# thallolang/thallo

Hardware: AMD Instinct MI355X
Metric: pcg_iters_per_sec (higher is better)
Workload: dtype f32

## Files before the change

include/thallo_hip.h:

```cpp
#ifndef THALLO_HIP_H
#define THALLO_HIP_H

#ifdef __cplusplus
extern "C" {
#endif

typedef void* thallo_stream_t;

#define THALLO_HIP_MAX_PARTIALS 1024

typedef struct thallo_sum_t {
    const float* partials;
    int          count;
} thallo_sum_t;

typedef struct thallo_segs_t {
    long off[8];
    long len[8];
    int  n;
} thallo_segs_t;

#define THALLO_DIST_MAX_WORLD 8
#define THALLO_DIST_CTL_WORDS 16
typedef struct thallo_dist_t {
    unsigned long long* mail;
    unsigned long long* peer_mail[THALLO_DIST_MAX_WORLD];
    float*    peer_r[2];
    long      peer_off_o[2];
    long      peer_off_a[2];
    unsigned* ctl;
    int       world, rank;
} thallo_dist_t;

typedef struct thallo_fin_t {
    thallo_sum_t alphaN;
    unsigned*    tickets;
    float*       alphaD_word;
    float*       betaN_word;
} thallo_fin_t;

typedef struct thallo_prev_t {
    const float*  alphaD_partials;
    const double* s12_partials;
    int           count;
    float*        alphaD_word;
    float*        betaN_word;
} thallo_prev_t;

long thallo_hip_vector_elems(long n_unknowns);
int  thallo_hip_device_cu_count(void);


int thallo_hip_pcg_step2(float* r, const float* Ap, const float* pre, float* z, long n,
                         thallo_sum_t alphaN, thallo_sum_t alphaD, float* betaN_out, thallo_stream_t stream);

int thallo_hip_pcg_step2_ranges(float* r, const float* Ap, const float* pre, float* z,
                                long off0, long len0, long off1, long len1,
                                thallo_sum_t alphaN, thallo_sum_t alphaD, float* betaN_out, thallo_stream_t stream);

int thallo_hip_pcg_step2_full(float* delta, const float* p, float* r, const float* Ap, const float* pre,
                              float* z, const float* b, long n, thallo_sum_t alphaN, thallo_sum_t alphaD,
                              float* betaN_out, float* q_out, int lm, thallo_stream_t stream);

int thallo_hip_pcg_step3(float* p, const float* z, long n, thallo_sum_t betaN, thallo_sum_t alphaN,
                         int lm, thallo_stream_t stream);

int thallo_hip_pcg_pupdate(const float* z, const float* p_in, float* p_out, float* delta, long n, int first,
                           thallo_sum_t alphaN_prev, thallo_sum_t alphaD_prev, thallo_sum_t betaN_prev, thallo_stream_t stream);
int thallo_hip_pcg_pupdate_ranges(const float* z, const float* p_in, float* p_out, float* delta,
                                  long off0, long len0, long off1, long len1, int first,
                                  thallo_sum_t alphaN_prev, thallo_sum_t alphaD_prev, thallo_sum_t betaN_prev, thallo_stream_t stream);

int thallo_hip_lm_finalize_diagonal(const float* diag, float* SSq, float* CtC, float* pre, const float* r, float* b, float* z, long n,
                                    float radius, float min_lm_diagonal, float max_lm_diagonal, int save_ssq, int use_preconditioner,
                                    float* alphaN_out, thallo_stream_t stream);
int thallo_hip_lm_step1_finish(float* Ap, const float* CtC, const float* p, long n, float* alphaD_out, thallo_stream_t stream);
int thallo_hip_lm_step2_first_half(float* delta, const float* p, long n, thallo_sum_t alphaN, thallo_sum_t alphaD, thallo_stream_t stream);
int thallo_hip_lm_step2_second_half(float* r, const float* b, const float* Adelta, const float* pre, float* z, const float* delta, long n,
                                    float* betaN_out, float* q_out, thallo_stream_t stream);
int thallo_hip_pcg_init_finish(const float* r, const float* diag, float* pre, float* z, long n, int use_preconditioner,
                               float* alphaN_out, thallo_stream_t stream);
void thallo_hip_lm_set_gate(const unsigned* gate);
int thallo_hip_lm_state_reset(float* state, thallo_stream_t stream);
int thallo_hip_lm_zeta(thallo_sum_t q, int k, float q_tolerance, float* state, thallo_stream_t stream);
int thallo_hip_pcg_step2_full_zeta(float* delta, const float* p, float* r, const float* Ap, const float* pre,
                                   float* z, const float* b, long n, thallo_sum_t alphaN, thallo_sum_t alphaD,
                                   float* betaN_out, float* q_out, unsigned* tickets, int k, float q_tolerance, float* lm_state, thallo_stream_t stream);
int thallo_hip_dot(const float* a, const float* b, long n, float* out, thallo_stream_t stream);

int thallo_hip_linear_update(float* X, const float* delta, const float* p, long len,
                             thallo_sum_t alphaN, thallo_sum_t alphaD, thallo_stream_t stream);

int thallo_hip_slab_pack_iter(const float* vec, thallo_segs_t segs, const float* alphaD_partials, const double* s3_partials, int count, float* out, thallo_stream_t stream);
int thallo_hip_slab_unpack_iter(float* vec, thallo_segs_t top, const float* src_top, thallo_segs_t bot, const float* src_bot,
                                const float* gathered, long stride, int world, thallo_sum_t alphaN, float* alphaD_word, float* betaN_word, thallo_stream_t stream);
int thallo_hip_block_sums(const float* p, const float* Ap, const float* r, const float* pre, long n, float* alphaD_out, double* s3_out, thallo_stream_t stream);
int thallo_hip_shard_scalars(const float* gathered, long stride, int world, const float* alphaD_partials, const double* s3_partials, int count, thallo_sum_t alphaN,
                             float* alphaD_word, float* betaN_word, thallo_stream_t stream);
int thallo_hip_range_unpack(float* vec, thallo_segs_t first_rank_pieces, const float* gathered, long stride, long skip, int world, thallo_stream_t stream);
int thallo_hip_linear_update2(float* X, const float* delta, const float* p_older, thallo_sum_t alphaN_older, thallo_sum_t alphaD_older,
                              const float* p, thallo_sum_t alphaN, thallo_sum_t alphaD, long len, thallo_stream_t stream);
#define THALLO_HIP_MAX_UPDATE_TERMS 32
typedef struct { const float* p[THALLO_HIP_MAX_UPDATE_TERMS]; thallo_sum_t alphaN[THALLO_HIP_MAX_UPDATE_TERMS], alphaD[THALLO_HIP_MAX_UPDATE_TERMS]; int count; } thallo_update_terms_t;
int thallo_hip_linear_update_n(float* X, float* delta, thallo_update_terms_t terms, long len, int max_workgroups , thallo_stream_t stream);
int thallo_hip_linear_update_n_from_zero(float* X, float* delta, thallo_update_terms_t terms, long len, int max_workgroups, thallo_stream_t stream);
int thallo_hip_wave64_selftest(unsigned long long* out_ballot, unsigned* out_peers, float* sums4);
int thallo_hip_finish_sum(thallo_sum_t s, float* out, thallo_stream_t stream);
int thallo_hip_finish_sum_gated(thallo_sum_t s, float* out, const unsigned* gate, thallo_stream_t stream);

int thallo_hip_slab_pack(const float* vec, thallo_segs_t segs, thallo_sum_t sum, float* out, thallo_stream_t stream);
int thallo_hip_slab_unpack(float* vec, thallo_segs_t top, const float* src_top, thallo_segs_t bot, const float* src_bot,
                           const float* gathered, long stride, int world, float* sum_out, thallo_stream_t stream);

int thallo_hip_alpha_beta(thallo_sum_t alphaN, thallo_sum_t alphaD, thallo_sum_t betaN, float* out2,
                          thallo_stream_t stream);

int thallo_hip_lapimg_cost(int W, int H, const float* X, const float* A, float w_fit, int xguard,
                           float* cost_out, thallo_stream_t stream);
int thallo_hip_lapimg_pcg_init(int W, int H, const float* X, const float* A, float w_fit, int xguard,
                               float* r, float* z, float* p_prev, float* delta,
                               float* diag_out, float* alphaN_out, thallo_stream_t stream);
int thallo_hip_lapimg_apply_jtj(int W, int H, float w_fit, int xguard, const float* p, float* Ap, float* alphaD_out, thallo_stream_t stream);
int thallo_hip_lapimg_pcg_step1(int W, int H, float w_fit, int xguard,
                                const float* z, const float* p_in, float* p_out, float* delta, float* Ap,
                                int first, thallo_sum_t alphaN_prev, thallo_sum_t alphaD_prev, thallo_sum_t betaN_prev,
                                float* alphaD_out, thallo_stream_t stream);

int thallo_hip_iw_cost(int W, int H, int row0, int row1, const float* offset, const float* angle, const float* urshape,
                       const float* constraints, const float* mask, float w_fit, float w_reg,
                       float* cost_out, thallo_stream_t stream);
int thallo_hip_iw_pcg_init(int W, int H, int row0, int row1, const float* offset, const float* angle, const float* urshape,
                           const float* constraints, const float* mask, float w_fit, float w_reg,
                           float* r, float* pre, float* z, float* p_prev, float* delta,
                           float* cs, unsigned char* flags, float* diag_out, int* irregular_out, float* alphaN_out, thallo_stream_t stream);
int thallo_hip_iw_pcg_step1(int W, int H, int row0, int row1, const float* cs, const float* urshape, const unsigned char* flags,
                            float w_fit, float w_reg,
                            const float* z, const float* p_in, float* p_out, float* delta, float* Ap,
                            int mode, thallo_sum_t alphaN_prev, thallo_sum_t alphaD_prev, thallo_sum_t betaN_prev,
                            thallo_sum_t alphaN_prev2, thallo_sum_t alphaD_prev2,
                            const int* irregular, const float* r, float* alphaD_out, thallo_stream_t stream);
#define THALLO_IW_STEP1_MODE(k, batched) ((k) == 0 ? 1 : !(batched) ? 0 : ((k) & 1) ? 2 : 4)
#define THALLO_HIP_FIN_TICKET_WORDS 528
typedef struct thallo_iw_iter_t {
    int W, H, row0, row1;
    const float* cs;
    const float* urshape;
    const unsigned char* flags;
    const float* pre;
    const int* irregular;
    float w_fit, w_reg;
    const float* r_in;  float* r_out;
    const float* Ap_in; float* Ap_out;
    const float* p_in;  float* p_out;
    float* delta;
    int mode;
    thallo_sum_t alphaN_prev, alphaD_prev, betaN_prev, alphaN_prev2, alphaD_prev2;
    float* alphaD_out; double* s12_out;
    unsigned* fin_tickets; float* alphaD_word; float* betaN_word; int slot0;
    const thallo_dist_t* dist;
    const thallo_prev_t* prev;
    int prev_slot0; unsigned long long* gs;
} thallo_iw_iter_t;
unsigned thallo_hip_iw_iter_size(void);
enum { THALLO_IW_ITER_TILE = 0, THALLO_IW_ITER_MARCH = 1, THALLO_IW_ITER_MARCH_RC = 2 };
int thallo_hip_iw_pcg_iter(int kernel, const thallo_iw_iter_t* a, thallo_stream_t stream);
int thallo_hip_iw_march_rc_deferred_fits(int W, int rows);
int thallo_hip_iw_dist_finish_deferred(thallo_prev_t prev, int prev_slot0, thallo_sum_t alphaN_prev, thallo_dist_t d, unsigned long long* gs, thallo_stream_t stream);
void thallo_hip_march_rc_debug_set(int what, int value);
int thallo_hip_iw_urshape_irregular(int W, int H, const float* urshape, int* count_out, thallo_stream_t stream);
void thallo_hip_march_debug_set(int what, int value);
int  thallo_hip_iw_resident_rows(int W, int rows);
long thallo_hip_iw_resident_bytes(int W, int rows);
int  thallo_hip_iw_pcg_resident(int W, int H, int row0, int row1, const float* cs, const unsigned char* flags, float w_fit, float w_reg,
                                const float* r_in, const float* p_in, float* r_out, float* Ap_out, float* p_out, float* delta,
                                thallo_sum_t alphaN0, float* words, const int* irregular, float* X_offset, float* X_angle, void* xbuf, int L, thallo_stream_t stream);
int  thallo_hip_iw_resident_status(void* xbuf, int clear, int spin_ms, unsigned* pm, thallo_stream_t stream);
int  thallo_hip_iw_resident_rows_slab(int W, int rows, int below);
long thallo_hip_iw_resident_ghost_bytes(int W);
int  thallo_hip_iw_pcg_resident_dist(int W, int H, int row0, int row1, const float* cs, const unsigned char* flags, float w_fit, float w_reg,
                                     const float* r_in, const float* p_in, float* r_out, float* Ap_out, float* p_out, float* delta,
                                     thallo_sum_t alphaN0, float* words, const int* irregular, void* xbuf, thallo_dist_t d, long ghost_off, int slot0, int L, thallo_stream_t stream);
void thallo_hip_resident_debug_set(int what, int value);
int thallo_hip_iw_march_rows(int W, int rows);
int thallo_hip_iw_march_place(int W, int row0, int row1, int R, int grid, int* place);
int thallo_hip_iw_pcg_iter_finish(const float* alphaD_partials, const double* s12_partials, int count, thallo_sum_t alphaN,
                                  float* alphaD_word, float* betaN_word, thallo_stream_t stream);

int thallo_hip_iw_pcg_step2(int W, int H, int row0, int row1, const unsigned char* flags, float w_fit, float w_reg,
// ... 369 lines not shown
```

thallo_amd/csrc/energy_image_warping.hip:

```cpp
#include "iw_device.hpp"

using namespace thallo;

namespace {

constexpr int TW = 64, TH = 16, BLOCK = 256;
constexpr int LW = TW + 2, LH = TH + 2, LN = LW * LH;
constexpr int PER = TH / (BLOCK / TW);
constexpr int HALO = 2 * LW + 2 * TH;

inline Geo make_geo(int W, int H, int row0, int row1)
{
    Geo g; g.W = W; g.H = H; g.row0 = row0; g.row1 = row1;
    g.tx = (W + TW - 1) / TW; g.ty = (row1 - row0 + TH - 1) / TH; g.ntiles = g.tx * g.ty;
    return g;
}
inline bool rows_ok(int H, int row0, int row1) { return row0 >= 0 && row1 <= H && row0 < row1; }
inline int grid_for(const Geo& g, int per_cu)
{
    int cap = thallo_hip_device_cu_count() * per_cu;
    if (cap > THALLO_MAX_PARTIALS) cap = THALLO_MAX_PARTIALS;
    cap -= cap % 8;
    return g.ntiles < cap ? g.ntiles : cap;
}
// ... 228 lines not shown
        const long i = in_off ? off0 + j : off1 + (j - len0);
        float4 rv = ldf4(r + i, true);
        const float4 av = Ap[i];
        rv.x -= alpha * av.x; rv.y -= alpha * av.y; rv.z -= alpha * av.z; rv.w -= alpha * av.w;
        float4 m;
        if (grid) {
            if (in_off) {
                const unsigned f2 = reinterpret_cast<const unsigned short*>(flags)[i];
                float m0, m1, dummy;
                pre_from_flags((unsigned char)(f2 & 255), wf2, wr2, m0, dummy); pre_from_flags((unsigned char)(f2 >> 8), wf2, wr2, m1, dummy);
                m = make_float4(m0, m0, m1, m1);
            } else {
                const unsigned f4 = reinterpret_cast<const unsigned*>(flags)[i - N / 2];
                float d, a0, a1, a2, a3;
                pre_from_flags((unsigned char)(f4 & 255), wf2, wr2, d, a0); pre_from_flags((unsigned char)((f4 >> 8) & 255), wf2, wr2, d, a1);
                pre_from_flags((unsigned char)((f4 >> 16) & 255), wf2, wr2, d, a2); pre_from_flags((unsigned char)(f4 >> 24), wf2, wr2, d, a3);
                m = make_float4(a0, a1, a2, a3);
            }
        } else m = pre[i];
        const float4 zv = make_float4(m.x * rv.x, m.y * rv.y, m.z * rv.z, m.w * rv.w);
        stf4(r + i, rv, true);
        if (!grid) z[i] = zv;
        if (DIST) {
            const long jj = in_off ? j : j - len0, rowlen = in_off ? row_o4 : row_a4, total = in_off ? len0 : len1;
            if (jj < rowlen && dd.peer_r[0]) {
                float* dst = dd.peer_r[0] + (in_off ? dd.peer_off_o[0] : dd.peer_off_a[0]) + 4 * jj;
                st_sys(dst, rv.x); st_sys(dst + 1, rv.y); st_sys(dst + 2, rv.z); st_sys(dst + 3, rv.w);
            }
            if (jj >= total - rowlen && dd.peer_r[1]) {
                float* dst = dd.peer_r[1] + (in_off ? dd.peer_off_o[1] : dd.peer_off_a[1]) + 4 * (jj - (total - rowlen));
                st_sys(dst, rv.x); st_sys(dst + 1, rv.y); st_sys(dst + 2, rv.z); st_sys(dst + 3, rv.w);
            }
        }
        acc += zv.x * rv.x + zv.y * rv.y + zv.z * rv.z + zv.w * rv.w;
    }
    block_store_partial(acc, bN_out, red);
}

__global__ __launch_bounds__(BLOCK) void k_step2_iw_rows(float* __restrict__ r, const float* __restrict__ Ap, const float* __restrict__ pre, float* __restrict__ z,
                                                         long off0, long len0, long off1, long len1, thallo_sum_t aN, thallo_sum_t aD, float* __restrict__ bN_out)
{
    __shared__ float red[16];
    const float alpha = safe_div<false>(sum_partials(aN.partials, aN.count), sum_partials(aD.partials, aD.count));
    float acc = 0.0f;
    const long n = len0 + len1;
    for (long j = (long)blockIdx.x * BLOCK + threadIdx.x; j < n; j += (long)gridDim.x * BLOCK) {
        const long i = j < len0 ? off0 + j : off1 + (j - len0);
        const float rv = r[i] - alpha * Ap[i];
        const float zv = pre ? pre[i] * rv : rv;
        r[i] = rv; z[i] = zv;
        acc += zv * rv;
    }
    block_store_partial(acc, bN_out, red);
}

__global__ __launch_bounds__(BLOCK) void k_init(Geo g, const float2* __restrict__ off, const float* __restrict__ ang,
                                                const float2* __restrict__ ur, const float2* __restrict__ cons,
                                                const float* __restrict__ mask, float wf, float wr,
                                                float* __restrict__ r, float* __restrict__ pre, float* __restrict__ z,
                                                float* __restrict__ p_prev, float* __restrict__ delta,
                                                float2* __restrict__ cs, unsigned char* __restrict__ flags,
                                                float* __restrict__ diag_out, int* __restrict__ irregular, float* __restrict__ aN_out)
{
    __shared__ Tile T;
    __shared__ float red[16];
    const long N = (long)g.W * g.H;
    const float wr2 = wr * wr, wf2 = wf * wf;
    float acc = 0.0f;
    int bad = 0;
    for (TileSweep t(g.ntiles); t.valid(); t.next()) {
        const int x0 = (t.cur % g.tx) * TW, y0 = g.row0 + (t.cur / g.tx) * TH;
        for (int idx = threadIdx.x; idx < LN; idx += BLOCK) {
            const int ly = idx / LW, lx = idx - ly * LW;
            const int gx = x0 + lx - 1, gy = y0 + ly - 1;
            float ox = 0.f, oy = 0.f, cc = 1.f, ss = 0.f, uxx = 0.f, uyy = 0.f; unsigned char ff = 0;
            if (gx >= 0 && gx < g.W && gy >= 0 && gy < g.H) {
                const long pix = (long)gy * g.W + gx;
                const float2 o = off[pix]; const float2 u = ur[pix];
                ox = o.x; oy = o.y; uxx = u.x; uyy = u.y;
                sincosf(ang[pix], &ss, &cc);
                ff = mask[pix] == 0.0f ? 1 : 0;
                if ((gy < g.row0 || gy >= g.row1) && lx >= 1 && lx <= TW) {
                    cs[pix] = make_float2(cc, ss); flags[pix] = ff;
                    reinterpret_cast<float2*>(p_prev)[pix] = make_float2(0.f, 0.f); p_prev[2 * N + pix] = 0.f;
                }
            }
            T.px[idx] = ox; T.py[idx] = oy; T.c[idx] = cc; T.s[idx] = ss; T.ux[idx] = uxx; T.uy[idx] = uyy; T.f[idx] = ff;
        }
        __syncthreads();
        const int lx = (threadIdx.x % TW) + 1;
        const int gx = x0 + lx - 1;
        for (int k = 0; k < PER; ++k) {
            const int ly = (threadIdx.x / TW) * PER + k + 1;
            const int gy = y0 + ly - 1;
            const int i = ly * LW + lx;
            if (gx < g.W && gy < g.row1) {
                const long pix = (long)gy * g.W + gx;
                const unsigned char act = T.f[i] & 1;
                const bool bad_x = gx + 1 < g.W && (T.ux[i + 1] - T.ux[i] != 1.0f || T.uy[i + 1] - T.uy[i] != 0.0f);
                const bool bad_y = gy + 1 < g.H && (T.ux[i + LW] - T.ux[i] != 0.0f || T.uy[i + LW] - T.uy[i] != 1.0f);
                if (bad_x || bad_y) ++bad;
                float rx = 0.f, ry = 0.f, ra = 0.f, mx = 0.f, my = 0.f, ma = 0.f, dgo_raw = 0.f, dga_raw = 0.f;
                unsigned char fl = act;
                if (act) {
                    const float oxi = T.px[i], oyi = T.py[i], ci = T.c[i], si = T.s[i], uxi = T.ux[i], uyi = T.uy[i];
                    float jx = 0.f, jy = 0.f, ja = 0.f, dgo = 0.f, dga = 0.f;
                    int cnt = 0; bool unit = true;
                    const int nb[4] = { i + 1, i - 1, i + LW, i - LW };
#pragma unroll
                    for (int d = 0; d < 4; ++d) {
                        const int j = nb[d];
                        if (T.f[j] & 1) {
                            const float dux = uxi - T.ux[j], duy = uyi - T.uy[j];
                            unit = unit && dux == (d == 0 ? -1.0f : d == 1 ? 1.0f : 0.0f) && duy == (d == 2 ? -1.0f : d == 3 ? 1.0f : 0.0f);
                            ++cnt;
                            const float dox = oxi - T.px[j], doy = oyi - T.py[j];
                            const float eix = dox - (ci * dux - si * duy), eiy = doy - (si * dux + ci * duy);
                            const float cj = T.c[j], sj = T.s[j];
                            const float ejx = -dox + (cj * dux - sj * duy), ejy = -doy + (sj * dux + cj * duy);
                            const float gix = -si * dux - ci * duy, giy = ci * dux - si * duy;
                            jx += eix - ejx; jy += eiy - ejy;
                            ja -= gix * eix + giy * eiy;
                            dgo += 2.0f; dga += gix * gix + giy * giy;
                        }
                    }
                    jx *= wr2; jy *= wr2; ja *= wr2; dgo *= wr2; dga *= wr2;
                    if (unit) dga = (float)cnt * wr2;
                    fl |= (unsigned char)(cnt << 2);
                    const float2 cv = cons[pix];
                    if (cv.x >= 0.0f && cv.y >= 0.0f) {
                        fl |= 2;
                        jx += wf2 * (oxi - cv.x); jy += wf2 * (oyi - cv.y); dgo += wf2;
                    }
                    rx = -jx; ry = -jy; ra = -ja;
                    mx = guarded_invert(dgo); my = mx; ma = guarded_invert(dga);
                    dgo_raw = dgo; dga_raw = dga;
                }
                if (diag_out) {
                    reinterpret_cast<float2*>(diag_out)[pix] = make_float2(dgo_raw, dgo_raw); diag_out[2 * N + pix] = dga_raw;
                }
                reinterpret_cast<float2*>(r)[pix] = make_float2(rx, ry);  r[2 * N + pix] = ra;
                reinterpret_cast<float2*>(pre)[pix] = make_float2(mx, my); pre[2 * N + pix] = ma;
                const float zx = mx * rx, zy = my * ry, zaa = ma * ra;
                reinterpret_cast<float2*>(z)[pix] = make_float2(zx, zy);  z[2 * N + pix] = zaa;
                reinterpret_cast<float2*>(p_prev)[pix] = make_float2(0.f, 0.f); p_prev[2 * N + pix] = 0.f;
                if (delta) { reinterpret_cast<float2*>(delta)[pix] = make_float2(0.f, 0.f);  delta[2 * N + pix] = 0.f; }
                cs[pix] = make_float2(T.c[i], T.s[i]);
                flags[pix] = fl;
                acc += rx * zx + ry * zy + ra * zaa;
            }
        }
        __syncthreads();
    }
    if (irregular && bad) atomicAdd(irregular, bad);
    block_store_partial(acc, aN_out, red);
}

constexpr int CW = 64, CH = 4;
__global__ __launch_bounds__(BLOCK) void k_cost(int W, int H, int row0, int row1, int ctx, int ntiles,
                                                const float2* __restrict__ off, const float* __restrict__ ang,
                                                const float2* __restrict__ ur, const float2* __restrict__ cons,
                                                const float* __restrict__ mask, float wf, float wr, float* __restrict__ out)
{
    __shared__ float red[16];
    float acc = 0.0f;
    for (TileSweep t(ntiles); t.valid(); t.next()) {
        const int x = (t.cur % ctx) * CW + (threadIdx.x % CW), y = row0 + (t.cur / ctx) * CH + (threadIdx.x / CW);
        if (x < W && y < row1) {
            const long i = (long)y * W + x;
            if (mask[i] == 0.0f) {
                const float2 o = off[i]; const float2 u = ur[i];
                float si, ci; sincosf(ang[i], &si, &ci);
                float s2 = 0.f;
                const int dx[4] = { 1, -1, 0, 0 }, dy[4] = { 0, 0, 1, -1 };
#pragma unroll
                for (int d = 0; d < 4; ++d) {
                    const int xn = x + dx[d], yn = y + dy[d];
                    if (xn >= 0 && xn < W && yn >= 0 && yn < H) {
                        const long j = (long)yn * W + xn;
                        if (mask[j] == 0.0f) {
                            const float2 oj = off[j]; const float2 uj = ur[j];
                            const float dux = u.x - uj.x, duy = u.y - uj.y;
                            const float ex = wr * ((o.x - oj.x) - (ci * dux - si * duy));
                            const float ey = wr * ((o.y - oj.y) - (si * dux + ci * duy));
                            s2 += ex * ex + ey * ey;
                        }
                    }
                }
                const float2 cv = cons[i];
                if (cv.x >= 0.0f && cv.y >= 0.0f) {
                    const float fx = wf * (o.x - cv.x), fy = wf * (o.y - cv.y);
                    s2 += fx * fx + fy * fy;
                }
                acc += 0.5f * s2;
            }
        }
    }
    block_store_partial(acc, out, red);
}

#ifdef THALLO_MARCH_SWEEP
__device__ unsigned long long* g_stamps = nullptr;
#define IW_STAMP(k) do { if (threadIdx.x == 0 && g_stamps) g_stamps[blockIdx.x * 8 + (k)] = wall_clock64(); } while (0)
#else
#define IW_STAMP(k) do { } while (0)
#endif
struct TileI : Tile { float rx[LN], ry[LN], ra[LN]; };
struct OwnedI { float2 rv, av, pv, csv, uv, dv, ppv, mv; float ra, aa, pav, da, ppa, ma; unsigned char ff; };
struct HaloI { float2 rv, av, pv, csv, uv, mv; float ra, aa, pav, ma; unsigned char ff; };

template <bool GRID, int NT, bool DIST = false>
__device__ __forceinline__ void iter_body(TileI& T, float* red, double* redd, const Geo& g, const float2* __restrict__ cs, const float2* __restrict__ ur,
                                          const unsigned char* __restrict__ flags, const float* __restrict__ pre, float wf2, float wr2,
                                          const float* __restrict__ r_in, float* __restrict__ r_out, const float* __restrict__ A_in, float* __restrict__ A_out,
                                          const float* __restrict__ p_in, float* __restrict__ p_out, float* __restrict__ delta, int mode,
                                          thallo_sum_t aNp, thallo_sum_t aDp, thallo_sum_t bNp, thallo_sum_t aNpp, thallo_sum_t aDpp,
                                          float* __restrict__ aD_out, double* __restrict__ s12_out, int ntm, const thallo_dist_t* dd = nullptr,
                                          unsigned* __restrict__ fin_tickets = nullptr, float* __restrict__ aD_word = nullptr, float* __restrict__ bN_word = nullptr,
                                          int xslot = 0, PrevSums prev = PrevSums{ nullptr, nullptr, 0, nullptr, nullptr })
{
    constexpr int PER = TH / (NT / TW);
    const int first = mode & 1;
    const int dmode = first ? 1 : (mode >> 1) & 3;
    const bool nt_delta = ntm & 1, nt_ra = ntm & 2, nt_out = ntm & 4, nt_pin = ntm & 8, nt_pout = ntm & 16, nt_const = ntm & 32;
    const long N = (long)g.W * g.H;
    const float2* __restrict__ ro = reinterpret_cast<const float2*>(r_in);   const float* __restrict__ ra = r_in + 2 * N;
    const float2* __restrict__ ao = reinterpret_cast<const float2*>(A_in);   const float* __restrict__ aa = A_in + 2 * N;
    const float2* __restrict__ po = reinterpret_cast<const float2*>(p_in);   const float* __restrict__ pa = p_in + 2 * N;
// ... 404 lines not shown
```

thallo_amd/csrc/energy_image_warping_march.hip:

```cpp
#include "iw_march.hpp"

namespace thallo {
int g_march_rows = 0;
int g_march_cap = 0;
}

using namespace thallo;

namespace {

inline int check_launch() { hipError_t e = hipGetLastError(); return e == hipSuccess ? 0 : -(int)e; }

template <bool FIRST>
struct Raw {
    float4 ro, po, cs, ao;
    float2 ra, pa, aa;
    unsigned f;
};
struct RawD { float4 dlo, ppo; float2 dla, ppa; };
template <bool FIRST>
__device__ __forceinline__ void take(Raw<FIRST>& d, const Raw<FIRST>& s)
{
    take4(d.ro, s.ro); take2(d.ra, s.ra); take4(d.po, s.po); take2(d.pa, s.pa); take4(d.cs, s.cs); take1(d.f, s.f);
    if (!FIRST) { take4(d.ao, s.ao); take2(d.aa, s.aa); }
}
template <int DMODE>
__device__ __forceinline__ void take(RawD& d, const RawD& s)
{
    take4(d.dlo, s.dlo); take2(d.dla, s.dla);
    if (DMODE == 2) { take4(d.ppo, s.ppo); take2(d.ppa, s.ppa); }
}

struct Row { float px[2], py[2], pa[2], c[2], s[2], rx[2], ry[2], ra[2], mo[2], ma[2]; unsigned f; };

template <bool FIRST, int DMODE, int NTM, bool DIST, int OCC>
__global__ __launch_bounds__(MARCH_NT, OCC) void k_iter_march(MarchGeo g, const float* __restrict__ cs, const unsigned char* __restrict__ flags, float wf2, float wr2,
                                                         const float* __restrict__ r_in, float* __restrict__ r_out, const float* __restrict__ A_in, float* __restrict__ A_out,
                                                         const float* __restrict__ p_in, float* __restrict__ p_out, float* __restrict__ delta,
                                                         thallo_sum_t aNp, thallo_sum_t aDp, thallo_sum_t bNp, thallo_sum_t aNpp, thallo_sum_t aDpp,
                                                         float* __restrict__ aD_out, double* __restrict__ s12_out, const int* __restrict__ irregular,
                                                         thallo_dist_t dd, unsigned* __restrict__ fin_tickets, float* __restrict__ aD_word, float* __restrict__ bN_word, int xslot,
                                                         PrevSums prev)
{
    __shared__ float2 lut[32];
    __shared__ float red[16];
    __shared__ double redd[48];
    constexpr bool nt_delta = NTM & 1, nt_ra = NTM & 2, nt_out = NTM & 4, nt_pin = NTM & 8, nt_pout = NTM & 16, nt_const = NTM & 32;
    int irregular_word = 0;
    if (irregular != nullptr) irregular_word = irregular[0];
    fence_order();

    const int lane = threadIdx.x & 63, wave = threadIdx.x >> 6;
    const long N = (long)g.W * g.H;
    const int W2 = g.W >> 1;
    int strip, ya, yb;
    march_place(g, wave, strip, ya, yb);
    const bool work = ya < yb;
    const int x0 = strip * MARCH_USE - 2 + 2 * lane;
    const bool xin = x0 >= 0 && x0 < g.W;
    const bool xout = xin && lane >= 1 && lane <= 62;

    const float4* __restrict__ ro4 = reinterpret_cast<const float4*>(r_in);  const float2* __restrict__ ra2 = reinterpret_cast<const float2*>(r_in + 2 * N);
    const float4* __restrict__ ao4 = reinterpret_cast<const float4*>(A_in);  const float2* __restrict__ aa2 = reinterpret_cast<const float2*>(A_in + 2 * N);
    const float4* __restrict__ po4 = reinterpret_cast<const float4*>(p_in);  const float2* __restrict__ pa2 = reinterpret_cast<const float2*>(p_in + 2 * N);
    const float4* __restrict__ cs4 = reinterpret_cast<const float4*>(cs);
    const unsigned* __restrict__ f4 = reinterpret_cast<const unsigned*>(flags);
    float4* __restrict__ Ro4 = reinterpret_cast<float4*>(r_out);  float2* __restrict__ Ra2 = reinterpret_cast<float2*>(r_out + 2 * N);
    float4* __restrict__ Ao4 = reinterpret_cast<float4*>(A_out);  float2* __restrict__ Aa2 = reinterpret_cast<float2*>(A_out + 2 * N);
    float4* __restrict__ qo4 = reinterpret_cast<float4*>(p_out);  float2* __restrict__ qa2 = reinterpret_cast<float2*>(p_out + 2 * N);
    float4* __restrict__ dl4 = reinterpret_cast<float4*>(delta);  float2* __restrict__ dl2 = reinterpret_cast<float2*>(delta + 2 * N);

    fence_order();
    if (__builtin_amdgcn_readfirstlane(irregular_word) != 0) {
        if (blockIdx.x == 0 && threadIdx.x == 0 && aD_word) { aD_word[0] = __builtin_nanf(""); bN_word[0] = __builtin_nanf(""); }
        if (blockIdx.x == 0 && threadIdx.x == 0 && prev.count > 0) { prev.aD_word[0] = __builtin_nanf(""); prev.bN_word[0] = __builtin_nanf(""); }
        if (threadIdx.x == 0) { aD_out[blockIdx.x] = __builtin_nanf(""); }
        return;
    }
    if (threadIdx.x < 32) { float mo, ma; pre_from_flags((unsigned char)threadIdx.x, wf2, wr2, mo, ma); lut[threadIdx.x] = make_float2(mo, ma); }
    __syncthreads();

    float alpha = 0.0f, beta = 0.0f, alpha2 = 0.0f;
    constexpr bool SCALARS_IN_LOOP = DMODE != 2;
    const bool scal_writer = work && strip == 0 && ya == g.row0 && lane == 0;
    if (!FIRST && !SCALARS_IN_LOOP) {
        iteration_scalars<1>(aNp, aDp, bNp, prev, alpha, beta, scal_writer);
        alpha2 = safe_div<false>(sum_partials(aNpp.partials, aNpp.count), sum_partials(aDpp.partials, aDpp.count));
    }

    typedef Raw<FIRST> RawT;
    RawT slot[3]; RawD dsl[3];
    auto row_exists = [&](int t) { return t >= 0 && t < g.H; };
    auto row_owned = [&](int t) { return t >= g.row0 && t < g.row1; };
    const int xc = x0 < 0 ? 0 : x0 > g.W - 2 ? g.W - 2 : x0;
    auto issue = [&](RawT& s, int t) {
        const int tc = t < 0 ? 0 : t > g.H - 1 ? g.H - 1 : t;
        const long i2 = (long)tc * W2 + (xc >> 1);
        s.ro = ldf4(ro4 + i2, nt_ra); s.ra = ldf2(ra2 + i2, nt_ra);
        if (!FIRST) { s.ao = ldf4(ao4 + i2, nt_ra); s.aa = ldf2(aa2 + i2, nt_ra); }
        s.po = ldf4(po4 + i2, nt_pin); s.pa = ldf2(pa2 + i2, nt_pin);
        s.cs = ldf4(cs4 + i2, nt_const);
        s.f = nt_const ? __builtin_nontemporal_load(f4 + (i2 >> 1)) : f4[i2 >> 1];
    };
    auto issue_d = [&](RawD& s, int t) {
        const int td = t < ya ? ya : t > yb - 1 ? yb - 1 : t;
        const long j2 = (long)td * W2 + (xc >> 1);
        s.dlo = ldf4(dl4 + j2, nt_delta); s.dla = ldf2(dl2 + j2, nt_delta);
        if (DMODE == 2) { s.ppo = qo4[j2]; s.ppa = qa2[j2]; }
    };

    Row win[3];
#pragma unroll
    for (int i = 0; i < 3; ++i) {
#pragma unroll
        for (int q = 0; q < 2; ++q) { win[i].px[q] = 0.f; win[i].py[q] = 0.f; win[i].pa[q] = 0.f; win[i].c[q] = 1.f; win[i].s[q] = 0.f;
                                      win[i].rx[q] = 0.f; win[i].ry[q] = 0.f; win[i].ra[q] = 0.f; win[i].mo[q] = 0.f; win[i].ma[q] = 0.f; }
        win[i].f = 0u;
    }

    auto publish = [&](const RawT& s, const RawD& sd, int t, Row& wn) {
        const bool ok = xin && row_exists(t);
        float rx[2] = { s.ro.x, s.ro.z }, ry[2] = { s.ro.y, s.ro.w }, rq[2] = { s.ra.x, s.ra.y };
        if (!FIRST) {
            rx[0] = __builtin_fmaf(-alpha, s.ao.x, rx[0]); ry[0] = __builtin_fmaf(-alpha, s.ao.y, ry[0]);
            rx[1] = __builtin_fmaf(-alpha, s.ao.z, rx[1]); ry[1] = __builtin_fmaf(-alpha, s.ao.w, ry[1]);
            rq[0] = __builtin_fmaf(-alpha, s.aa.x, rq[0]); rq[1] = __builtin_fmaf(-alpha, s.aa.y, rq[1]);
        }
        const float ppx[2] = { s.po.x, s.po.z }, ppy[2] = { s.po.y, s.po.w }, ppq[2] = { s.pa.x, s.pa.y };
        const unsigned fl = ok ? (s.f >> (((((long)t * W2 + (x0 >> 1)) & 1) != 0) ? 16 : 0)) & 0xffffu : 0u;
        const float2 m0 = lut[fl & 31u], m1 = lut[(fl >> 8) & 31u];
        const float mo[2] = { m0.x, m1.x }, ma[2] = { m0.y, m1.y };
#pragma unroll
        for (int q = 0; q < 2; ++q) {
            wn.px[q] = ok ? mo[q] * rx[q] + beta * ppx[q] : 0.f; wn.py[q] = ok ? mo[q] * ry[q] + beta * ppy[q] : 0.f; wn.pa[q] = ok ? ma[q] * rq[q] + beta * ppq[q] : 0.f;
            wn.rx[q] = rx[q]; wn.ry[q] = ry[q]; wn.ra[q] = rq[q]; wn.mo[q] = mo[q]; wn.ma[q] = ma[q];
        }
        wn.c[0] = s.cs.x; wn.s[0] = s.cs.y; wn.c[1] = s.cs.z; wn.s[1] = s.cs.w; wn.f = fl;
        const bool mine = t >= ya && t < yb;
        if (ok && xout && (mine || !row_owned(t))) {
            const long i2 = (long)t * W2 + (x0 >> 1);
            stf4(Ro4 + i2, make_float4(rx[0], ry[0], rx[1], ry[1]), nt_out); stf2(Ra2 + i2, make_float2(rq[0], rq[1]), nt_out);
            stf4(qo4 + i2, make_float4(wn.px[0], wn.py[0], wn.px[1], wn.py[1]), nt_pout); stf2(qa2 + i2, make_float2(wn.pa[0], wn.pa[1]), nt_pout);
            if (DMODE != 1 && mine) {
                float4 d = sd.dlo; float2 da = sd.dla;
                if (DMODE == 2) {
                    d.x = __builtin_fmaf(alpha2, sd.ppo.x, d.x); d.y = __builtin_fmaf(alpha2, sd.ppo.y, d.y);
                    d.z = __builtin_fmaf(alpha2, sd.ppo.z, d.z); d.w = __builtin_fmaf(alpha2, sd.ppo.w, d.w);
                    da.x = __builtin_fmaf(alpha2, sd.ppa.x, da.x); da.y = __builtin_fmaf(alpha2, sd.ppa.y, da.y);
                }
                d.x = __builtin_fmaf(alpha, ppx[0], d.x); d.y = __builtin_fmaf(alpha, ppy[0], d.y);
                d.z = __builtin_fmaf(alpha, ppx[1], d.z); d.w = __builtin_fmaf(alpha, ppy[1], d.w);
                da.x = __builtin_fmaf(alpha, ppq[0], da.x); da.y = __builtin_fmaf(alpha, ppq[1], da.y);
                stf4(dl4 + i2, d, nt_delta); stf2(dl2 + i2, da, nt_delta);
            }
        }
    };

    float acc = 0.0f; double s0 = 0.0, s1 = 0.0, s2 = 0.0;
    auto stencil = [&](int y, const Row& wm, const Row& wc, const Row& wn) {
        float ax[2], ay[2], av[2], am[2], ac[2], an[2], wfm[2], wfc[2], wfn[2];
        flag_masks(wm.f, wf2, am, wfm); flag_masks(wc.f, wf2, ac, wfc); flag_masks(wn.f, wf2, an, wfn);
        jtjp_pair(wm, wc, wn, wm, wc, wn, am, ac, an, wfc, wr2, ax, ay, av);
        if (xout) {
#pragma unroll
            for (int q = 0; q < 2; ++q)
                iter_sums_pixel(wc.px[q], wc.py[q], wc.pa[q], ax[q], ay[q], av[q], wc.rx[q], wc.ry[q], wc.ra[q], wc.mo[q], wc.ma[q], acc, s0, s1, s2);
            const long i2 = (long)y * W2 + (x0 >> 1);
            stf4(Ao4 + i2, make_float4(ax[0], ay[0], ax[1], ay[1]), nt_out); stf2(Aa2 + i2, make_float2(av[0], av[1]), nt_out);
            if (DIST) {
#pragma unroll
                for (int k = 0; k < 2; ++k) {
                    if (y == (k == 0 ? g.row0 : g.row1 - 1) && dd.peer_r[k]) {
                        float* d2 = dd.peer_r[k] + dd.peer_off_o[k] + 2 * x0;
                        st_sys(d2, ax[0]); st_sys(d2 + 1, ay[0]); st_sys(d2 + 2, ax[1]); st_sys(d2 + 3, ay[1]);
                        float* d1 = dd.peer_r[k] + dd.peer_off_a[k] + x0;
                        st_sys(d1, av[0]); st_sys(d1 + 1, av[1]);
                    }
                }
            }
        }
    };

    if (work) {
        const int t_first = ya - 1, t_last = yb;
#pragma unroll
        for (int j = 0; j < 3; ++j) { slot[j] = RawT{}; dsl[j] = RawD{}; }
        for (int t0 = t_first - 3; t0 <= t_last; t0 += 3) {
            if (!FIRST && SCALARS_IN_LOOP && t0 == t_first) iteration_scalars<1>(aNp, aDp, bNp, prev, alpha, beta, scal_writer);
#pragma unroll
            for (int j = 0; j < 3; ++j) {
                const int t = t0 + j;
                Row& wn = win[(j + 2) % 3]; Row& wc = win[(j + 1) % 3]; Row& wm = win[j % 3];
                RawT cur; RawD curd = RawD{};
                take(cur, slot[j]);
                if (DMODE != 1) take<DMODE>(curd, dsl[j]);
                fence_order();
                issue(slot[j], t + 3 > t_last ? t_last : t + 3);
                if (DMODE != 1) issue_d(dsl[(j + 2) % 3], t + 2);
                fence_order();
                if (t >= t_first && t <= t_last) publish(cur, curd, t, wn);
                if (t - 1 >= ya && t <= t_last) stencil(t - 1, wm, wc, wn);
            }
        }
    }
    iter_tail<MARCH_NT, DIST>(acc, s0, s1, s2, red, redd, aD_out, s12_out, bNp, &dd, fin_tickets, aD_word, bN_word, xslot);
}

__global__ __launch_bounds__(256) void k_urshape_check(int W, int H, const float2* __restrict__ ur, int* __restrict__ bad_out)
{
    int bad = 0;
    const long N = (long)W * H;
    for (long i = (long)blockIdx.x * blockDim.x + threadIdx.x; i < N; i += (long)gridDim.x * blockDim.x) {
        const int x = (int)(i % W), y = (int)(i / W);
        const float2 u = ur[i];
        bool off = false;
        if (x + 1 < W) { const float2 v = ur[i + 1]; off = v.x - u.x != 1.0f || v.y - u.y != 0.0f; }
        if (y + 1 < H) { const float2 v = ur[i + W]; off = off || v.x - u.x != 0.0f || v.y - u.y != 1.0f; }
        if (off) ++bad;
    }
    if (bad) atomicAdd(bad_out, bad);
}

constexpr int MARCH_OCC = 2;

template <bool DIST>
int launch_march_as(const thallo_iw_iter_t& a, hipStream_t stream)
{
    const IterForm f(a);
    const int R = march_pick_rows(a.W, a.row1 - a.row0);
    if (R <= 0) return -(int)hipErrorNotSupported;
    const MarchGeo g = make_march_geo(a.W, a.H, a.row0, a.row1, R);
    const int grid = (g.total + 7) / 8 * 8;
    if (grid > THALLO_MAX_PARTIALS) return -(int)hipErrorInvalidValue;
    const bool first = a.mode & 1;
    const int dmode = first ? 1 : (a.mode >> 1) & 3;
    const float wf2 = a.w_fit * a.w_fit, wr2 = a.w_reg * a.w_reg;
#define MARCH_LAUNCH(F, DM) hipLaunchKernelGGL((k_iter_march<F, DM, MARCH_NTM, DIST, MARCH_OCC>), dim3(grid), dim3(MARCH_NT), 0, stream, g, a.cs, a.flags, wf2, wr2, \
        a.r_in, a.r_out, a.Ap_in, a.Ap_out, a.p_in, a.p_out, a.delta, a.alphaN_prev, f.aDp, f.bNp, a.alphaN_prev2, a.alphaD_prev2, a.alphaD_out, a.s12_out, a.irregular, f.d, \
        f.tickets, f.aD_word, f.bN_word, f.xslot, f.prev)
    if (DIST && dmode == 2) return -(int)hipErrorInvalidValue;
    if (first) MARCH_LAUNCH(true, 1);
    else if (dmode == 1) MARCH_LAUNCH(false, 1);
    else if (dmode == 2) { if constexpr (!DIST) MARCH_LAUNCH(false, 2); }
    else MARCH_LAUNCH(false, 0);
#undef MARCH_LAUNCH
    int e = check_launch(); return e ? e : grid;
}

}

int thallo::launch_march(const thallo_iw_iter_t& a, hipStream_t stream)
{
    if ((a.W & 1) || a.W < 2 || !a.Ap_out || (!(a.mode & 1) && !a.Ap_in)) return -(int)hipErrorInvalidValue;
    if (a.dist && a.gs) return -(int)hipErrorNotSupported;
    return !a.dist ? launch_march_as<false>(a, stream) : launch_march_as<true>(a, stream);
}

extern "C" {
int thallo_hip_iw_urshape_irregular(int W, int H, const float* urshape, int* count_out, thallo_stream_t stream)
{
    if (W < 1 || H < 1 || !urshape || !count_out) return -(int)hipErrorInvalidValue;
    if (hipMemsetAsync(count_out, 0, sizeof(int), (hipStream_t)stream) != hipSuccess) return -(int)hipErrorInvalidValue;
    int grid = thallo_hip_device_cu_count() * 8;
    const long want = ((long)W * H + 255) / 256;
    if (want < grid) grid = (int)want;
    hipLaunchKernelGGL(k_urshape_check, dim3(grid), dim3(256), 0, (hipStream_t)stream, W, H, (const float2*)urshape, count_out);
    return check_launch();
}


void thallo_hip_march_debug_set(int what, int value)
{
    if (what == 0) g_march_rows = value;
    if (what == 6) g_march_cap = value;
}

int thallo_hip_iw_march_rows(int W, int rows)
{
    if (W < 2 || (W & 1) || rows < 1) return 0;
    return march_pick_rows(W, rows);
}

}
```

thallo_amd/csrc/pcg_kernels.hip:

```cpp
#include "device_common.hpp"
#include "../../include/thallo_hip.h"

using namespace thallo;

namespace {

constexpr int BLOCK = 256;

inline int flat_grid(long n4, int cus)
{
    long want = (n4 + BLOCK - 1) / BLOCK;
    long cap = (long)cus * 4;
    if (cap > THALLO_MAX_PARTIALS) cap = THALLO_MAX_PARTIALS;
    if (cap >= 8) cap -= cap % 8;
    if (want > cap) want = cap;
    if (want < 1) want = 1;
    return (int)want;
}

int g_cus = 0;
int g_nt2 = 3;
int cu_count()
{
    if (!g_cus) {
// ... 409 lines not shown
        const float4 x = a[i], y = b[i];
        acc += x.x * y.x + x.y * y.y + x.z * y.z + x.w * y.w;
    }
    block_store_partial(acc, out, red);
}

template <bool HAS_P>
__global__ __launch_bounds__(BLOCK) void k_linear_update(float* __restrict__ X, const float* __restrict__ delta,
                                                          const float* __restrict__ p, long len,
                                                          thallo_sum_t aN, thallo_sum_t aD)
{
    float alpha = 0.0f;
    if (HAS_P) alpha = safe_div<false>(sum_partials(aN.partials, aN.count), sum_partials(aD.partials, aD.count));
    for (long i = (long)blockIdx.x * BLOCK + threadIdx.x; i < len; i += (long)gridDim.x * BLOCK) {
        float d = delta[i];
        if (HAS_P) d = __builtin_fmaf(alpha, p[i], d);
        X[i] = X[i] + d;
    }
}

__global__ __launch_bounds__(BLOCK) void k_linear_update2(float* __restrict__ X, const float* __restrict__ delta,
                                                           const float* __restrict__ p0, thallo_sum_t aN0, thallo_sum_t aD0,
                                                           const float* __restrict__ p1, thallo_sum_t aN1, thallo_sum_t aD1, long len)
{
    const float a0 = safe_div<false>(sum_partials(aN0.partials, aN0.count), sum_partials(aD0.partials, aD0.count));
    const float a1 = safe_div<false>(sum_partials(aN1.partials, aN1.count), sum_partials(aD1.partials, aD1.count));
    for (long i = (long)blockIdx.x * BLOCK + threadIdx.x; i < len; i += (long)gridDim.x * BLOCK) {
        float d = delta[i];
        d = __builtin_fmaf(a0, p0[i], d);
        d = __builtin_fmaf(a1, p1[i], d);
        X[i] = X[i] + d;
    }
}

__device__ __forceinline__ float2 sum_partials_pair(const float* __restrict__ pa, int na, const float* __restrict__ pb, int nb)
{
    const int lane = threadIdx.x & (THALLO_WAVE - 1);
    constexpr int PER = THALLO_MAX_PARTIALS / THALLO_WAVE;
    float va[PER], vb[PER];
#pragma unroll
    for (int k = 0; k < PER; ++k) { const int i = lane + k * THALLO_WAVE; va[k] = i < na ? pa[i] : 0.0f; }
#pragma unroll
    for (int k = 0; k < PER; ++k) { const int i = lane + k * THALLO_WAVE; vb[k] = i < nb ? pb[i] : 0.0f; }
    float sa = 0.0f, sb = 0.0f;
#pragma unroll
    for (int k = 0; k < PER; ++k) sa += va[k];
#pragma unroll
    for (int k = 0; k < PER; ++k) sb += vb[k];
    sa = wave_sum_all(sa); sb = wave_sum_all(sb);
    const float wa = __builtin_bit_cast(float, __builtin_amdgcn_readfirstlane(__builtin_bit_cast(int, va[0])));
    const float wb = __builtin_bit_cast(float, __builtin_amdgcn_readfirstlane(__builtin_bit_cast(int, vb[0])));
    return make_float2(na == 1 ? wa : sa, nb == 1 ? wb : sb);
}
__device__ __forceinline__ const float* wave_uniform_ptr(const float* p, int lane)
{
    const unsigned long long b = (unsigned long long)reinterpret_cast<uintptr_t>(p);
    const unsigned lo = (unsigned)__builtin_amdgcn_readlane((int)(unsigned)b, lane), hi = (unsigned)__builtin_amdgcn_readlane((int)(unsigned)(b >> 32), lane);
    return reinterpret_cast<const float*>((uintptr_t)(((unsigned long long)hi << 32) | lo));
}
__device__ __forceinline__ void update_alphas(const thallo_update_terms_t& T, float* __restrict__ al)
{
    const int lane = threadIdx.x & (THALLO_WAVE - 1);
    const int wave = __builtin_amdgcn_readfirstlane((int)(threadIdx.x / THALLO_WAVE));
    const bool mine = lane < T.count;
    const int jl = mine ? lane : 0;
    const float* pn = T.alphaN[jl].partials; const float* pd = T.alphaD[jl].partials;
    const int cn = T.alphaN[jl].count, cd = T.alphaD[jl].count;
    const bool words = cn == 1 && cd == 1;
    if (wave == 0 && mine && words) al[lane] = safe_div<false>(pn[0], pd[0]);
    unsigned lists = (unsigned)__ballot(mine && !words);
    lists &= 0x11111111u << wave;
    while (lists) {
        const int j = __builtin_ctz(lists);
        lists &= lists - 1;
        const float2 s = sum_partials_pair(wave_uniform_ptr(pn, j), __builtin_amdgcn_readlane(cn, j), wave_uniform_ptr(pd, j), __builtin_amdgcn_readlane(cd, j));
        if (lane == 0) al[j] = safe_div<false>(s.x, s.y);
    }
}

__device__ __forceinline__ void fma4(float4& d, float a, const float4& q)
{
    d.x = __builtin_fmaf(a, q.x, d.x); d.y = __builtin_fmaf(a, q.y, d.y); d.z = __builtin_fmaf(a, q.z, d.z); d.w = __builtin_fmaf(a, q.w, d.w);
}
__device__ __forceinline__ void apply_terms4(float4& d, int j, long i, const thallo_update_terms_t& T, const float* al)
{
    for (; j + 8 <= T.count; j += 8) {
        float4 q[8];
#pragma unroll
        for (int u = 0; u < 8; ++u) q[u] = ldf4(reinterpret_cast<const float4*>(T.p[j + u]) + i, true);
#pragma unroll
        for (int u = 0; u < 8; ++u) fma4(d, al[j + u], q[u]);
    }
    for (; j + 4 <= T.count; j += 4) {
        float4 q[4];
#pragma unroll
        for (int u = 0; u < 4; ++u) q[u] = ldf4(reinterpret_cast<const float4*>(T.p[j + u]) + i, true);
#pragma unroll
        for (int u = 0; u < 4; ++u) fma4(d, al[j + u], q[u]);
    }
    for (; j < T.count; ++j) fma4(d, al[j], ldf4(reinterpret_cast<const float4*>(T.p[j]) + i, true));
}
__device__ __forceinline__ void store_update4(float* __restrict__ X, float* __restrict__ delta, long i, const float4& d)
{
    if (X) { float4 x = reinterpret_cast<const float4*>(X)[i]; x.x = x.x + d.x; x.y = x.y + d.y; x.z = x.z + d.z; x.w = x.w + d.w; reinterpret_cast<float4*>(X)[i] = x; }
    else reinterpret_cast<float4*>(delta)[i] = d;
}

template <bool V4, bool ZERO>
__global__ __launch_bounds__(BLOCK) void k_linear_update_n(float* __restrict__ X, float* __restrict__ delta, thallo_update_terms_t T, long len)
{
    __shared__ float al[THALLO_HIP_MAX_UPDATE_TERMS];
    const long i0 = (long)blockIdx.x * BLOCK + threadIdx.x, stride = (long)gridDim.x * BLOCK;
    if (V4) {
        const long n4 = len >> 2;
        const bool have = i0 < n4, eight = T.count >= 8;
        float4 d = make_float4(0.0f, 0.0f, 0.0f, 0.0f), q[8];
        if (have) {
            if (!ZERO) d = reinterpret_cast<const float4*>(delta)[i0];
            if (eight) {
#pragma unroll
                for (int u = 0; u < 8; ++u) q[u] = ldf4(reinterpret_cast<const float4*>(T.p[u]) + i0, true);
            }
        }
        update_alphas(T, al);
        __syncthreads();
        if (have) {
            if (eight) {
#pragma unroll
                for (int u = 0; u < 8; ++u) fma4(d, al[u], q[u]);
            }
            apply_terms4(d, eight ? 8 : 0, i0, T, al);
            store_update4(X, delta, i0, d);
        }
        for (long i = i0 + stride; i < n4; i += stride) {
            float4 e = make_float4(0.0f, 0.0f, 0.0f, 0.0f);
            if (!ZERO) e = reinterpret_cast<const float4*>(delta)[i];
            apply_terms4(e, 0, i, T, al);
            store_update4(X, delta, i, e);
        }
    } else {
        float d = 0.0f;
        if (!ZERO && i0 < len) d = delta[i0];
        update_alphas(T, al);
        __syncthreads();
        for (long i = i0; i < len; i += stride) {
            if (i != i0) d = ZERO ? 0.0f : delta[i];
            for (int j = 0; j < T.count; ++j) d = __builtin_fmaf(al[j], T.p[j][i], d);
            if (X) X[i] = X[i] + d; else delta[i] = d;
        }
    }
}

__global__ __launch_bounds__(BLOCK) void k_slab_pack(const float* __restrict__ vec, thallo_segs_t segs, thallo_sum_t s, float* __restrict__ out)
{
    if (blockIdx.x == 0 && s.count > 0) {
        const float v = sum_partials(s.partials, s.count);
        if (threadIdx.x == 0) out[0] = v;
    }
    long base = 1;
    for (int k = 0; k < segs.n; ++k) {
        for (long i = (long)blockIdx.x * BLOCK + threadIdx.x; i < segs.len[k]; i += (long)gridDim.x * BLOCK) out[base + i] = vec[segs.off[k] + i];
        base += segs.len[k];
    }
}

__global__ __launch_bounds__(BLOCK) void k_slab_unpack(float* __restrict__ vec, thallo_segs_t top, const float* __restrict__ src_top,
                                                        thallo_segs_t bot, const float* __restrict__ src_bot,
                                                        const float* __restrict__ gathered, long stride, int world, float* __restrict__ sum_out)
{
    if (blockIdx.x == 0 && threadIdx.x == 0 && sum_out) {
        float v = 0.0f;
        for (int r = 0; r < world; ++r) v += gathered[(long)r * stride];
        sum_out[0] = v;
    }
    if (src_top) {
        long base = 0;
        for (int k = 0; k < top.n; ++k) {
            for (long i = (long)blockIdx.x * BLOCK + threadIdx.x; i < top.len[k]; i += (long)gridDim.x * BLOCK) vec[top.off[k] + i] = src_top[base + i];
            base += top.len[k];
        }
    }
    if (src_bot) {
        long base = 0;
        for (int k = 0; k < bot.n; ++k) {
            for (long i = (long)blockIdx.x * BLOCK + threadIdx.x; i < bot.len[k]; i += (long)gridDim.x * BLOCK) vec[bot.off[k] + i] = src_bot[base + i];
            base += bot.len[k];
        }
    }
}

template <bool HAS_PRE>
__global__ __launch_bounds__(BLOCK) void k_block_sums(const float4* __restrict__ p, const float4* __restrict__ Ap, const float4* __restrict__ r, const float4* __restrict__ pre,
                                                       long n4, float* __restrict__ aD_out, double* __restrict__ s3_out)
{
    __shared__ float red[16];
    __shared__ double redd[3 * BLOCK / 64];
    float acc = 0.0f; Sums3 sm;
    for (long i = (long)blockIdx.x * BLOCK + threadIdx.x; i < n4; i += (long)gridDim.x * BLOCK) {
        const float4 pv = p[i], av = Ap[i], rv = r[i];
        float4 m = make_float4(1.f, 1.f, 1.f, 1.f);
        if (HAS_PRE) m = pre[i];
        acc += pv.x * av.x + pv.y * av.y + pv.z * av.z + pv.w * av.w;
        sm.add(m.x, rv.x, av.x); sm.add(m.y, rv.y, av.y); sm.add(m.z, rv.z, av.z); sm.add(m.w, rv.w, av.w);
    }
    block_store_partial(acc, aD_out, red);
    block_store_sums3(sm, s3_out, redd);
}
__global__ __launch_bounds__(64) void k_shard_scalars(const float* __restrict__ gathered, long stride, int world, const float* __restrict__ aD_part, const double* __restrict__ s3_part,
                                                      int nb, thallo_sum_t aN, int count_only_first, float* __restrict__ out_a, float* __restrict__ out_b)
{
    const int lane = threadIdx.x;
    float ad = 0.0f; double q[3] = { 0.0, 0.0, 0.0 };
    for (int r = 0; r < world; ++r) {
        const float* m = gathered + (long)r * stride;
        ad += m[0];
        if (!count_only_first)
            for (int j = 0; j < 3; ++j) {
                const unsigned long long b = ((unsigned long long)__float_as_uint(m[1 + 2 * j]) << 32) | (unsigned long long)__float_as_uint(m[2 + 2 * j]);
                q[j] += __longlong_as_double((long long)b);
            }
    }
    ad += sum_partials(aD_part, nb);
    if (count_only_first) { if (lane == 0) out_a[0] = ad; return; }
    double n = 0.0, a = 0.0, b = 0.0;
    for (int i = lane; i < nb; i += THALLO_WAVE) { n += s3_part[3 * i]; a += s3_part[3 * i + 1]; b += s3_part[3 * i + 2]; }
    n = q[0] + wave_sum_all_f64(n); a = q[1] + wave_sum_all_f64(a); b = q[2] + wave_sum_all_f64(b);
    const float an = sum_partials(aN.partials, aN.count);
    const float alpha = safe_div<false>(an, ad);
    double bn = n - 2.0 * (double)alpha * a + (double)alpha * (double)alpha * b;
// ... 353 lines not shown
    int e = check_launch(); return e ? e : grid;
}
int thallo_hip_lm_step1_finish(float* Ap, const float* CtC, const float* p, long n, float* aD_out, thallo_stream_t stream)
{
    const long n4 = (n + 3) / 4; const int grid = flat_grid(n4, cu_count());
    hipLaunchKernelGGL(k_lm_step1_finish, dim3(grid), dim3(BLOCK), 0, (hipStream_t)stream, (float4*)Ap, (const float4*)CtC, (const float4*)p, n4, aD_out, g_gate);
    int e = check_launch(); return e ? e : grid;
}
int thallo_hip_lm_step2_first_half(float* delta, const float* p, long n, thallo_sum_t aN, thallo_sum_t aD, thallo_stream_t stream)
{
    const long n4 = (n + 3) / 4; const int grid = flat_grid(n4, cu_count());
    hipLaunchKernelGGL(k_lm_step2_first, dim3(grid), dim3(BLOCK), 0, (hipStream_t)stream, (float4*)delta, (const float4*)p, n4, aN, aD, g_gate);
    int e = check_launch(); return e ? e : grid;
}
int thallo_hip_lm_step2_second_half(float* r, const float* b, const float* Adelta, const float* pre, float* z, const float* delta, long n,
                                    float* bN_out, float* q_out, thallo_stream_t stream)
{
    const long n4 = (n + 3) / 4; const int grid = flat_grid(n4, cu_count());
    hipLaunchKernelGGL(k_lm_step2_second, dim3(grid), dim3(BLOCK), 0, (hipStream_t)stream, (float4*)r, (const float4*)b, (const float4*)Adelta,
                       (const float4*)pre, (float4*)z, (const float4*)delta, n4, bN_out, q_out, g_gate);
    int e = check_launch(); return e ? e : grid;
}
int thallo_hip_pcg_init_finish(const float* r, const float* diag, float* pre, float* z, long n, int use_preconditioner,
                               float* aN_out, thallo_stream_t stream)
{
    const long n4 = (n + 3) / 4; const int grid = flat_grid(n4, cu_count());
    hipLaunchKernelGGL(k_init_finish, dim3(grid), dim3(BLOCK), 0, (hipStream_t)stream, (const float4*)r, (const float4*)diag, (float4*)pre, (float4*)z, n4,
                       use_preconditioner, aN_out);
    int e = check_launch(); return e ? e : grid;
}
int thallo_hip_dot(const float* a, const float* b, long n, float* out, thallo_stream_t stream)
{
    const long n4 = (n + 3) / 4; const int grid = flat_grid(n4, cu_count());
    hipLaunchKernelGGL(k_dot, dim3(grid), dim3(BLOCK), 0, (hipStream_t)stream, (const float4*)a, (const float4*)b, n4, out);
    int e = check_launch(); return e ? e : grid;
}

int thallo_hip_linear_update(float* X, const float* delta, const float* p, long len,
                             thallo_sum_t aN, thallo_sum_t aD, thallo_stream_t stream)
{
    const int grid = flat_grid(len, cu_count());
    hipStream_t s = (hipStream_t)stream;
    if (p) hipLaunchKernelGGL(k_linear_update<true>, dim3(grid), dim3(BLOCK), 0, s, X, delta, p, len, aN, aD);
    else   hipLaunchKernelGGL(k_linear_update<false>, dim3(grid), dim3(BLOCK), 0, s, X, delta, p, len, aN, aD);
    int e = check_launch();
    return e ? e : grid;
}

int thallo_hip_linear_update2(float* X, const float* delta, const float* p_older, thallo_sum_t aN0, thallo_sum_t aD0,
                              const float* p, thallo_sum_t aN1, thallo_sum_t aD1, long len, thallo_stream_t stream)
{
    if (!p_older || !p) return -(int)hipErrorInvalidValue;
    const int grid = flat_grid(len, cu_count());
    hipLaunchKernelGGL(k_linear_update2, dim3(grid), dim3(BLOCK), 0, (hipStream_t)stream, X, delta, p_older, aN0, aD0, p, aN1, aD1, len);
    int e = check_launch();
    return e ? e : grid;
}

static int linear_update_n(bool zero, float* X, float* delta, const thallo_update_terms_t& terms, long len, int max_workgroups, thallo_stream_t stream)
{
    if (!delta || len < 0 || terms.count < 0 || terms.count > THALLO_HIP_MAX_UPDATE_TERMS) return -(int)hipErrorInvalidValue;
    bool v4 = !(len & 3) && !(((uintptr_t)X | (uintptr_t)delta) & 15);
    for (int j = 0; j < terms.count; ++j) {
        if (!terms.p[j] || !terms.alphaN[j].partials || !terms.alphaD[j].partials || terms.alphaN[j].count < 1 || terms.alphaD[j].count < 1) return -(int)hipErrorInvalidValue;
        if ((uintptr_t)terms.p[j] & 15) v4 = false;
    }
    if (len == 0 || (terms.count == 0 && !X && !zero)) return 0;
    int grid = flat_grid(v4 ? len >> 2 : len, 2 * cu_count());
    if (max_workgroups > 0 && grid > max_workgroups) grid = max_workgroups;
    auto kernel = v4 ? (zero ? k_linear_update_n<true, true> : k_linear_update_n<true, false>) : (zero ? k_linear_update_n<false, true> : k_linear_update_n<false, false>);
    hipLaunchKernelGGL(kernel, dim3(grid), dim3(BLOCK), 0, (hipStream_t)stream, X, delta, terms, len);
    int e = check_launch();
    return e ? e : grid;
}
int thallo_hip_linear_update_n(float* X, float* delta, thallo_update_terms_t terms, long len, int max_workgroups, thallo_stream_t stream)
{
    return linear_update_n(false, X, delta, terms, len, max_workgroups, stream);
}
int thallo_hip_linear_update_n_from_zero(float* X, float* delta, thallo_update_terms_t terms, long len, int max_workgroups, thallo_stream_t stream)
{
    return linear_update_n(true, X, delta, terms, len, max_workgroups, stream);
}

int thallo_hip_finish_sum(thallo_sum_t sum, float* out, thallo_stream_t stream)
{
    hipLaunchKernelGGL(k_finish_sum, dim3(1), dim3(64), 0, (hipStream_t)stream, sum, out);
    return check_launch();
}

int thallo_hip_finish_sum_gated(thallo_sum_t sum, float* out, const unsigned* gate, thallo_stream_t stream)
{
    if (!gate || !out || !sum.partials) return -(int)hipErrorInvalidValue;
    hipLaunchKernelGGL(k_finish_sum_gated, dim3(1), dim3(64), 0, (hipStream_t)stream, sum, out, gate);
    return check_launch();
}

int thallo_hip_slab_pack(const float* vec, thallo_segs_t segs, thallo_sum_t sum, float* out, thallo_stream_t stream)
{
    if (segs.n < 0 || segs.n > 8) return -(int)hipErrorInvalidValue;
    hipLaunchKernelGGL(k_slab_pack, dim3(8), dim3(BLOCK), 0, (hipStream_t)stream, vec, segs, sum, out);
    return check_launch();
}

int thallo_hip_slab_unpack(float* vec, thallo_segs_t top, const float* src_top, thallo_segs_t bot, const float* src_bot,
                           const float* gathered, long stride, int world, float* sum_out, thallo_stream_t stream)
{
    if (top.n < 0 || top.n > 8 || bot.n < 0 || bot.n > 8) return -(int)hipErrorInvalidValue;
    hipLaunchKernelGGL(k_slab_unpack, dim3(8), dim3(BLOCK), 0, (hipStream_t)stream, vec, top, src_top, bot, src_bot, gathered, stride, world, sum_out);
    return check_launch();
}

int thallo_hip_block_sums(const float* p, const float* Ap, const float* r, const float* pre, long n, float* aD_out, double* s3_out, thallo_stream_t stream)
{
    if (!p || !Ap || !r || !aD_out || !s3_out || n < 0 || (n & 3)) return -(int)hipErrorInvalidValue;
    const long n4 = n / 4; const int grid = flat_grid(n4 ? n4 : 1, cu_count());
    if (pre) hipLaunchKernelGGL(k_block_sums<true>, dim3(grid), dim3(BLOCK), 0, (hipStream_t)stream, (const float4*)p, (const float4*)Ap, (const float4*)r, (const float4*)pre, n4, aD_out, s3_out);
    else     hipLaunchKernelGGL(k_block_sums<false>, dim3(grid), dim3(BLOCK), 0, (hipStream_t)stream, (const float4*)p, (const float4*)Ap, (const float4*)r, (const float4*)pre, n4, aD_out, s3_out);
    int e = check_launch(); return e ? e : grid;
}
int thallo_hip_shard_scalars(const float* gathered, long stride, int world, const float* aD_partials, const double* s3_partials, int count, thallo_sum_t alphaN,
                             float* alphaD_word, float* betaN_word, thallo_stream_t stream)
{
    if (!gathered || world < 1 || stride < 1 || !aD_partials || count < 0 || count > THALLO_MAX_PARTIALS || !alphaD_word) return -(int)hipErrorInvalidValue;
    const int only_first = betaN_word == nullptr;
    if (!only_first && (!s3_partials || alphaN.count < 1)) return -(int)hipErrorInvalidValue;
    hipLaunchKernelGGL(k_shard_scalars, dim3(1), dim3(64), 0, (hipStream_t)stream, gathered, stride, world, aD_partials, s3_partials, count, alphaN, only_first, alphaD_word, betaN_word);
    return check_launch();
}

int thallo_hip_range_unpack(float* vec, thallo_segs_t first_rank_pieces, const float* gathered, long stride, long skip, int world, thallo_stream_t stream)
{
    if (!vec || !gathered || first_rank_pieces.n < 1 || first_rank_pieces.n > 8 || world < 1 || stride < 1 || skip < 0) return -(int)hipErrorInvalidValue;
    long len = 0; for (int j = 0; j < first_rank_pieces.n; ++j) len += first_rank_pieces.len[j];
    int grid = (int)((len + BLOCK - 1) / BLOCK); if (grid > 64) grid = 64; if (grid < 1) grid = 1;
    hipLaunchKernelGGL(k_range_unpack, dim3(grid), dim3(BLOCK), 0, (hipStream_t)stream, vec, first_rank_pieces, gathered, stride, skip, world);
    return check_launch();
}

static bool units_ok(const thallo_units_t& u, bool unpack)
{
    if (u.n < 0 || u.nplanes < 1 || u.nplanes > 8 || (u.n > 0 && (!u.units || (unpack && !u.src)))) return false;
    for (int k = 0; k < u.nplanes; ++k) if (u.len[k] < 1 || u.base[k] < 0) return false;
    return true;
}
static int units_grid(const thallo_units_t& u) { long t = 0; for (int k = 0; k < u.nplanes; ++k) t += u.len[k]; t *= u.n; int g = (int)((t + BLOCK - 1) / BLOCK); return g > 64 ? 64 : g < 1 ? 1 : g; }
int thallo_hip_units_pack(const float* vec, thallo_units_t u, thallo_sum_t sum, float* out, thallo_stream_t stream)
{
    if (!units_ok(u, false) || !out || (u.n > 0 && !vec) || sum.count < 0 || (sum.count > 0 && !sum.partials)) return -(int)hipErrorInvalidValue;
    hipLaunchKernelGGL(k_units_pack, dim3(units_grid(u)), dim3(BLOCK), 0, (hipStream_t)stream, vec, u, sum, out);
    return check_launch();
}
int thallo_hip_units_unpack(float* vec, thallo_units_t u, const float* gathered, long stride, int world, float* sum_out, thallo_stream_t stream)
{
    if (!units_ok(u, true) || !gathered || (u.n > 0 && !vec) || stride < 1 || world < 1) return -(int)hipErrorInvalidValue;
    hipLaunchKernelGGL(k_units_unpack, dim3(units_grid(u)), dim3(BLOCK), 0, (hipStream_t)stream, vec, u, gathered, stride, world, sum_out);
    return check_launch();
}
int thallo_hip_units_pack_iter(const float* vec, thallo_units_t u, const float* aD_partials, const double* s3_partials, int count, float* out, thallo_stream_t stream)
{
    if (!units_ok(u, false) || !aD_partials || !s3_partials || count < 1 || count > THALLO_MAX_PARTIALS || !out || (u.n > 0 && !vec)) return -(int)hipErrorInvalidValue;
    hipLaunchKernelGGL(k_units_pack_iter, dim3(units_grid(u)), dim3(BLOCK), 0, (hipStream_t)stream, vec, u, aD_partials, s3_partials, count, out);
    return check_launch();
}
int thallo_hip_units_unpack_iter(float* vec, thallo_units_t u, const float* gathered, long stride, int world, thallo_sum_t alphaN,
                                 float* alphaD_word, float* betaN_word, thallo_stream_t stream)
{
// ... 28 lines not shown
```

thallo_amd/csrc/plugin.hpp:

```cpp
#pragma once
#include <hip/hip_runtime.h>
#include <string>
#include <vector>
#include <map>
#include "../../include/thallo_hip.h"

namespace thallo {

class ReducedCameraSystem;

void set_error(const char* fmt, ...);
const char* last_error();
const char* env_switch(const char* name);

class KernelTimer {
public:
    struct Stat { std::string name; long launches = 0; long samples = 0; double total_ms = 0; double sq_ms = 0;
                  std::vector<std::pair<hipEvent_t, hipEvent_t>> pending;
                  long ksamples = 0; double ktotal_ms = 0; std::vector<std::pair<hipEvent_t, hipEvent_t>> kpending; };
    int period = 0;
    bool invasive = false;
    ~KernelTimer();
    int  begin(const char* name, hipStream_t s);
    void end(int slot, hipStream_t s);
// ... 5 lines not shown
    std::vector<hipEvent_t> open_;
    std::vector<hipEvent_t> pool_;
    hipEvent_t k0_ = nullptr, k1_ = nullptr;
    hipEvent_t get_event();
};

struct LaunchCtx {
    hipStream_t stream = nullptr;
    KernelTimer* timer = nullptr;
    const unsigned* gate = nullptr;
    const float* lm_ctc = nullptr;
    float *lm_defer_aD_word = nullptr, *lm_defer_bN_word = nullptr;
    int lm_q_in = 0, lm_q_out = 0;
    float* lm_reset_bn_word = nullptr;
};

struct TimedLaunch {
    LaunchCtx& c; int slot;
    TimedLaunch(LaunchCtx& ctx, const char* name) : c(ctx), slot(ctx.timer ? ctx.timer->begin(name, ctx.stream) : -1) {}
    ~TimedLaunch() { if (slot >= 0) c.timer->end(slot, c.stream); }
};

struct SolverVectors {
    long n = 0, n_alloc = 0;
    float *delta = nullptr, *r = nullptr, *z = nullptr, *Ap = nullptr, *pre = nullptr;
    float *p[2] = { nullptr, nullptr };
    float *b = nullptr, *Adelta = nullptr, *CtC = nullptr, *SSq = nullptr, *prevX = nullptr, *diag = nullptr;
    float *r2 = nullptr, *Ap2 = nullptr;
    double* s12 = nullptr;
    double* s12b = nullptr;
    double* s12buf(int i) { return i ? s12b : s12; }
    unsigned* fin_tickets = nullptr;
    float* rbuf(int i) { return i ? r2 : r; }
    float* Abuf(int i) { return i ? Ap2 : Ap; }
};

struct UnknownImage { int param_index; long n_floats; };

struct Vectors64 { long n = 0, n_alloc = 0; double *delta = nullptr, *r = nullptr, *z = nullptr, *Ap = nullptr, *pre = nullptr, *p = nullptr;
                   double* diag = nullptr; };
class EnergyPlugin64 {
public:
    virtual ~EnergyPlugin64() {}
    virtual int cost64(struct LaunchCtx&, double* partials_out) = 0;
    virtual int pcg_init64(struct LaunchCtx&, Vectors64&, double* alphaN_partials) = 0;
    virtual int apply_jtj64(struct LaunchCtx&, Vectors64&, const double* p, double* Ap, double* alphaD_partials) = 0;
    virtual double* unknown_ptr64(int k) = 0;
};

class EnergyPlugin {
public:
    virtual ~EnergyPlugin() {}
    virtual const char* name() const = 0;
    virtual EnergyPlugin64* f64() { return nullptr; }
    virtual const char* schedule_name() const { return "matrix-free"; }
    virtual long n_unknowns() const = 0;
    virtual const std::vector<UnknownImage>& unknown_images() const = 0;
    virtual bool use_preconditioner() const = 0;
    virtual int bind(void** params) = 0;
    virtual int prepare(LaunchCtx&) { return 0; }
    virtual int cost(LaunchCtx&, float* cost_out) = 0;
    virtual int pcg_init(LaunchCtx&, SolverVectors&, int cur, float* alphaN_out) = 0;
    virtual int apply_jtj(LaunchCtx&, const float* p, float* Ap, float* alphaD_out) = 0;
    virtual bool apply_adds_ctc() const { return false; }
    virtual bool lm_one_kernel() const { return false; }
    virtual bool lm_iter_defers_finish() const { return false; }
    virtual bool lm_iter_after_reset() const { return false; }
    virtual int lm_reset_residual(LaunchCtx&, SolverVectors&, float* ) { return -1; }
    virtual bool lm_one_kernel_slab() const { return false; }
    virtual int pcg_iter_lm(LaunchCtx&, SolverVectors&, int , bool , thallo_sum_t , thallo_sum_t , thallo_sum_t , float* ,
                            const thallo_fin_t&, float* , int , float ) { return -1; }
    virtual bool init_folds_lm_diagonal() const { return false; }
    virtual int pcg_init_lm(LaunchCtx&, SolverVectors&, int , float , float , float , int , float* ) { return -1; }
    virtual bool lm_model_cost_one_launch() const { return false; }
    virtual int lm_model_cost(LaunchCtx&, SolverVectors&, const float* , const float* , int , const float* , int ,
                              float* , float* , bool ) { return -1; }
    virtual bool apply_folds_pupdate() const { return false; }
    virtual int apply_jtj_pupdate(LaunchCtx&, const float* , const float* , float* , float* , float* , bool ,
                                  thallo_sum_t , thallo_sum_t ) { return -1; }
    virtual int pcg_step1(LaunchCtx&, SolverVectors&, int cur, bool first,
                          thallo_sum_t aN_prev, thallo_sum_t aD_prev, thallo_sum_t bN_prev, float* alphaD_out) = 0;
    virtual bool batches_delta() const { return false; }
    virtual bool takes_any_p_plane() const { return false; }
    virtual bool init_takes_null_delta() const { return false; }
    virtual bool persist_ok() const { return false; }
    virtual int pcg_persist(struct LaunchCtx&, SolverVectors&, float* const* planes, int n_planes, int k0, int k1, float* parts, int slots, int B, int nb_prev, thallo_sum_t alphaN_prev) { return -1; }
    virtual int pcg_step1_mode(LaunchCtx& c, SolverVectors& v, int cur, int mode, thallo_sum_t aN_prev, thallo_sum_t aD_prev, thallo_sum_t bN_prev,
                               thallo_sum_t, thallo_sum_t, float* alphaD_out)
    { return pcg_step1(c, v, cur, (mode & 1) != 0, aN_prev, aD_prev, bN_prev, alphaD_out); }
    virtual bool apply_returns_sums() const { return false; }
    virtual int apply_jtj_sums(LaunchCtx&, SolverVectors&, const float* , float* , float* , const thallo_fin_t& ) { return -1; }
    virtual bool one_kernel_iteration() const { return false; }
    virtual bool dist_flat_form() const { return !one_kernel_iteration(); }
    virtual bool one_kernel_slab() const { return false; }
    virtual int pcg_iter(LaunchCtx&, SolverVectors&, int , int , thallo_sum_t, thallo_sum_t, thallo_sum_t, thallo_sum_t, thallo_sum_t, float* ,
                         float* , float* ) { return -1; }
    virtual int pcg_iter_finish(LaunchCtx&, SolverVectors&, const float* , int , thallo_sum_t , float* , float* ) { return -1; }
    virtual bool iter_defers_finish() const { return false; }
    virtual int pcg_iter_deferred(LaunchCtx&, SolverVectors&, int , int , thallo_sum_t , thallo_sum_t , thallo_sum_t ,
                                  const thallo_prev_t& , float* , double* ) { return -1; }
    virtual int pcg_iter_finish_from(LaunchCtx&, const float* , const double* , int , thallo_sum_t ,
                                     float* , float* ) { return -1; }
    virtual bool resident_ok() const { return false; }
    virtual int  pcg_resident(LaunchCtx&, SolverVectors&, int , thallo_sum_t , float* ) { return -1; }
    virtual bool resident_updates_unknowns() const { return false; }
    virtual bool resident_lm_ok() const { return false; }
    virtual int  pcg_resident_lm(LaunchCtx&, SolverVectors&, int , thallo_sum_t , float* , float* , float , float* , float* ) { return -1; }
    virtual int  resident_status(LaunchCtx&, int , unsigned* ) { return 0; }
    virtual void resident_disable() {}
    virtual bool dist_defers_finish() const { return false; }
    virtual int  pcg_iter_dist_deferred(LaunchCtx&, SolverVectors&, int , int , thallo_sum_t , thallo_sum_t , thallo_sum_t , thallo_sum_t , thallo_sum_t ,
                                        const thallo_prev_t& , int , unsigned long long* , const thallo_dist_t&, float* , double* ) { return -1; }
    virtual int  pcg_iter_dist_finish(LaunchCtx&, const thallo_prev_t& , int , thallo_sum_t , const thallo_dist_t&, unsigned long long* ) { return -1; }
    virtual bool dist_batches_delta() const { return false; }
    virtual bool resident_slab_ok() const { return false; }
    virtual long resident_ghost_bytes() const { return 0; }
    virtual int  pcg_resident_dist(LaunchCtx&, SolverVectors&, int , thallo_sum_t , float* , const thallo_dist_t&, long , int ) { return -1; }
    virtual int pcg_step2(LaunchCtx& c, SolverVectors& v, thallo_sum_t aN, thallo_sum_t aD, float* betaN_out)
    {
        TimedLaunch t(c, "PCGStep2");
        return thallo_hip_pcg_step2(v.r, v.Ap, use_preconditioner() ? v.pre : nullptr, v.z, v.n, aN, aD, betaN_out, c.stream);
    }
    virtual bool block_precond_ok() const { return false; }
    virtual thallo_block_regions_t block_regions() const { thallo_block_regions_t r; r.n = 0; return r; }
    virtual int block_diag(LaunchCtx&, float* ) { return -1; }
    virtual ReducedCameraSystem* reduced_system() { return nullptr; }
    virtual bool hold_ok() const { return false; }
    virtual void hold_to_internal(int , const unsigned char* , unsigned char* ) const {}
    virtual void prior_to_internal(int , const float* , float* ) const {}
    virtual bool robust_ok() const { return false; }
    virtual int robust_prepare(int , float ) { return 0; }
    virtual long robust_weights(LaunchCtx&, float* , long ) { return -1; }
    virtual float* unknown_ptr(int k) = 0;
    virtual void unknowns_changed() {}
    virtual void unknowns_written() { unknowns_changed(); }
    virtual void forbid_renumbering() {}
    virtual bool direct_solve() const { return false; }
    virtual int  solve_direct(LaunchCtx&, SolverVectors&) { return -1; }
    virtual bool supports_row_slabs() const { return false; }
    virtual int  set_row_slab(int , int ) { return -1; }
    virtual int  slab_ghost_rows() const { return 1; }
    virtual bool slab_returns_sums() const { return apply_returns_sums(); }
    virtual bool slab_setup_ok() const { return true; }
    virtual const char* slab_setup_error() const { return ""; }
    virtual int  set_slab_global(int , int ) { return 0; }
    virtual int  slab_width() const { return 0; }
    virtual bool slab_grid_ok() const { return false; }
    virtual unsigned char* slab_flags() { return nullptr; }
    virtual long range_units() const { return 0; }
    virtual int  set_owned_range(long , long ) { return -1; }
    virtual long shared_block_offset() const { return 0; }
    virtual long shared_block_floats() const { return 0; }
    virtual int  shared_split_slots() const { return 0; }
    virtual int  pcg_iter_dist(LaunchCtx&, SolverVectors&, int , int , thallo_sum_t, thallo_sum_t, thallo_sum_t, thallo_sum_t, thallo_sum_t,
                               const thallo_dist_t&, float* , int , float* , float* ) { return -1; }
};

struct DeviceBuffer {
    void* ptr = nullptr; size_t bytes = 0;
    int alloc(size_t n);
    int upload(const std::vector<int>& h);
    void release();
    ~DeviceBuffer() { release(); }
};

struct ProblemSpec {
// ... 16 lines not shown
```

thallo_amd/csrc/plugins.cpp:

```cpp
#include "plugin.hpp"
#include "ba_reduced.hpp"
#include "ba_structure.hpp"
#ifdef THALLO_RESEARCH
#include "probe/thallo_hip_research.h"
#endif
#include <algorithm>
#include <cstdio>
#include <cstring>
#include <cstdlib>

namespace thallo {

int DeviceBuffer::alloc(size_t n)
{
    release();
    if (n == 0) return 0;
    hipError_t e = hipMalloc(&ptr, n);
    if (e != hipSuccess) { ptr = nullptr; set_error("hipMalloc(%zu) failed: %s", n, hipGetErrorString(e)); return -(int)e; }
    bytes = n;
    e = hipMemset(ptr, 0, n);
    return e == hipSuccess ? 0 : -(int)e;
}
int DeviceBuffer::upload(const std::vector<int>& h)
{
// ... 186 lines not shown
            }
            if (need > 0) { resident_ = whole; resident_slab_ = true; }
        }
        persist_ = false;
#ifdef THALLO_RESEARCH
        const char* ep = env_switch("THALLO_PERSIST");
        if (march_rc_ && whole && !resident_broken_ && ep && ep[0] == '1' && thallo_hip_iw_march_persist_rows(W, H) > 0) {
            const long need = thallo_hip_iw_march_persist_bytes();
            if ((long)xpst.bytes < need && xpst.alloc((size_t)need)) { set_error("image_warping: out of device memory for the persistent loop's exchange buffer"); return -1; }
            persist_ = true;
        }
#endif
        return 0;
    }
    bool supports_row_slabs() const override { return true; }
    int set_row_slab(int row0, int row1) override
    {
        if (row0 < 0 || row1 > H || row0 >= row1 || (W & 3)) { set_error("image_warping: row slab [%d,%d) of %d rows, W = %d (W %% 4 must be 0)", row0, row1, H, W); return -1; }
        row0_ = row0; row1_ = row1; return 0;
    }
    int slab_width() const override { return W; }
    bool slab_grid_ok() const override { return grid_; }
    unsigned char* slab_flags() override { return (unsigned char*)flags.ptr; }
private:
    thallo_iw_iter_t iter_block(SolverVectors& v, int cur, int mode, thallo_sum_t aN, thallo_sum_t aD, thallo_sum_t bN, thallo_sum_t aN2, thallo_sum_t aD2, float* out, double* s12_out) const
    {
        thallo_iw_iter_t a = {};
        a.W = W; a.H = H; a.row0 = row0_; a.row1 = row1_;
        a.cs = (const float*)cs.ptr; a.urshape = urshape; a.flags = (const unsigned char*)flags.ptr; a.pre = v.pre; a.irregular = (const int*)irregular.ptr;
        a.w_fit = w_fit; a.w_reg = w_reg;
        a.r_in = v.rbuf(cur); a.r_out = v.rbuf(cur ^ 1); a.Ap_in = v.Abuf(cur); a.Ap_out = v.Abuf(cur ^ 1); a.p_in = v.p[cur]; a.p_out = v.p[cur ^ 1]; a.delta = v.delta; a.mode = mode;
        a.alphaN_prev = aN; a.alphaD_prev = aD; a.betaN_prev = bN; a.alphaN_prev2 = aN2; a.alphaD_prev2 = aD2;
        a.alphaD_out = out; a.s12_out = s12_out;
        return a;
    }
    int run_iter(LaunchCtx& c, const thallo_iw_iter_t& a)
    {
        TimedLaunch t(c, "PCGIteration");
        const int kernel = march_rc_ && !(a.mode & 1) ? THALLO_IW_ITER_MARCH_RC : march_ ? THALLO_IW_ITER_MARCH : THALLO_IW_ITER_TILE;
        return thallo_hip_iw_pcg_iter(kernel, &a, c.stream);
    }
public:
    int pcg_iter_dist(LaunchCtx& c, SolverVectors& v, int cur, int mode, thallo_sum_t aN, thallo_sum_t aD, thallo_sum_t bN, thallo_sum_t aN2, thallo_sum_t aD2,
                      const thallo_dist_t& d, float* out, int slot0, float* aD_word, float* bN_word) override
    {
        thallo_iw_iter_t a = iter_block(v, cur, mode, aN, aD, bN, aN2, aD2, out, v.s12);
        a.dist = &d; a.fin_tickets = v.fin_tickets; a.slot0 = slot0; a.alphaD_word = aD_word; a.betaN_word = bN_word;
        return run_iter(c, a);
    }
    bool dist_defers_finish() const override { return march_rc_ && march_ && thallo_hip_iw_march_rc_deferred_fits(W, row1_ - row0_) != 0; }
    int pcg_iter_dist_deferred(LaunchCtx& c, SolverVectors& v, int cur, int mode, thallo_sum_t aN, thallo_sum_t aD, thallo_sum_t bN, thallo_sum_t aN2, thallo_sum_t aD2,
                               const thallo_prev_t& prev, int prev_slot0, unsigned long long* gs, const thallo_dist_t& d, float* out, double* s12_out) override
    {
        thallo_iw_iter_t a = iter_block(v, cur, mode, aN, aD, bN, aN2, aD2, out, s12_out);
        a.dist = &d;
        if (!(mode & 1)) { a.prev = &prev; a.prev_slot0 = prev_slot0; a.gs = gs; }
        return run_iter(c, a);
    }
    int pcg_iter_dist_finish(LaunchCtx& c, const thallo_prev_t& prev, int prev_slot0, thallo_sum_t aN, const thallo_dist_t& d, unsigned long long* gs) override
    { TimedLaunch t(c, "PCGScalars"); return thallo_hip_iw_dist_finish_deferred(prev, prev_slot0, aN, d, gs, c.stream); }
    float* unknown_ptr(int k) override { return k == 0 ? offset : angle; }
    int cost(LaunchCtx& c, float* out) override
    { TimedLaunch t(c, "computeCost"); return thallo_hip_iw_cost(W, H, row0_, row1_, offset, angle, urshape, constraints, mask, w_fit, w_reg, out, c.stream); }
    int pcg_init(LaunchCtx& c, SolverVectors& v, int cur, float* aN) override
    {
        TimedLaunch t(c, "PCGInit1");
        return thallo_hip_iw_pcg_init(W, H, row0_, row1_, offset, angle, urshape, constraints, mask, w_fit, w_reg,
                                      v.r, v.pre, v.z, v.p[cur], v.delta, (float*)cs.ptr, (unsigned char*)flags.ptr, v.diag, (int*)irregular.ptr, aN, c.stream);
    }
    int apply_jtj(LaunchCtx& c, const float* p, float* Ap, float* out) override
    {
        TimedLaunch t(c, "PCGStep1");
        return thallo_hip_iw_apply_jtj(W, H, row0_, row1_, (const float*)cs.ptr, urshape, (const unsigned char*)flags.ptr, w_fit, w_reg, p, Ap, (const int*)irregular.ptr, out, c.stream);
    }
    int pcg_step1(LaunchCtx& c, SolverVectors& v, int cur, bool first, thallo_sum_t aN, thallo_sum_t aD, thallo_sum_t bN, float* out) override
    {
        TimedLaunch t(c, "PCGStep1");
        const thallo_sum_t none = { nullptr, 0 };
        return thallo_hip_iw_pcg_step1(W, H, row0_, row1_, (const float*)cs.ptr, urshape, (const unsigned char*)flags.ptr, w_fit, w_reg,
                                       v.z, v.p[cur], v.p[cur ^ 1], v.delta, v.Ap, first ? 1 : 0, aN, aD, bN, none, none, (const int*)irregular.ptr, v.r, out, c.stream);
    }
    bool batches_delta() const override { return true; }
    bool init_takes_null_delta() const override { return true; }
    bool takes_any_p_plane() const override { return march_; }
    bool persist_ok() const override { return persist_; }
#ifdef THALLO_RESEARCH
    int pcg_persist(LaunchCtx& c, SolverVectors& v, float* const* planes, int n_planes, int k0, int k1, float* parts, int slots, int B, int nb_prev, thallo_sum_t alphaN_prev) override
    {
        TimedLaunch t(c, "PCGLoopPersistent");
        return thallo_hip_iw_pcg_march_persist(W, H, (const float*)cs.ptr, (const unsigned char*)flags.ptr, w_fit, w_reg, v.rbuf(0), v.rbuf(1), planes, n_planes, k0, k1,
                                               parts, slots, B, v.s12, v.s12b, nb_prev, alphaN_prev, (const int*)irregular.ptr, xpst.ptr, c.stream);
    }
#endif
    bool dist_batches_delta() const override { return march_rc_; }
    bool one_kernel_iteration() const override { return true; }
    int pcg_iter(LaunchCtx& c, SolverVectors& v, int cur, int mode, thallo_sum_t aN, thallo_sum_t aD, thallo_sum_t bN, thallo_sum_t aN2, thallo_sum_t aD2, float* out,
                 float* aD_word, float* bN_word) override
    {
        thallo_iw_iter_t a = iter_block(v, cur, mode, aN, aD, bN, aN2, aD2, out, v.s12);
        a.fin_tickets = aD_word ? v.fin_tickets : nullptr; a.alphaD_word = aD_word; a.betaN_word = bN_word;
        return run_iter(c, a);
    }
    int pcg_iter_finish(LaunchCtx& c, SolverVectors& v, const float* part, int count, thallo_sum_t aN, float* aD_word, float* bN_word) override
    {
        TimedLaunch t(c, "PCGScalars");
        return thallo_hip_iw_pcg_iter_finish(part, v.s12, count, aN, aD_word, bN_word, c.stream);
    }
    bool resident_ok() const override { return resident_; }
    int pcg_resident(LaunchCtx& c, SolverVectors& v, int L, thallo_sum_t aN0, float* words) override
    {
        TimedLaunch t(c, "PCGLoopResident");
        return thallo_hip_iw_pcg_resident(W, H, row0_, row1_, (const float*)cs.ptr, (const unsigned char*)flags.ptr, w_fit, w_reg, v.rbuf(0), v.p[0],
                                          v.rbuf(L & 1), v.Abuf(L & 1), v.p[L & 1], v.delta, aN0, words, (const int*)irregular.ptr,
                                          resident_updates_unknowns() ? offset : nullptr, resident_updates_unknowns() ? angle : nullptr, xres.ptr, L, c.stream);
    }
    bool resident_updates_unknowns() const override { const char* e = env_switch("THALLO_IW_RESIDENT_FOLD"); return resident_ && !(e && e[0] == '0'); }
    bool resident_slab_ok() const override { return resident_slab_; }
    long resident_ghost_bytes() const override { return (W & 1) ? 0 : thallo_hip_iw_resident_ghost_bytes(W); }
    int pcg_resident_dist(LaunchCtx& c, SolverVectors& v, int L, thallo_sum_t aN0, float* words, const thallo_dist_t& d, long ghost_off, int slot0) override
    {
        if (!resident_slab_) return -(int)hipErrorNotSupported;
        TimedLaunch t(c, "PCGLoopResident");
        return thallo_hip_iw_pcg_resident_dist(W, H, row0_, row1_, (const float*)cs.ptr, (const unsigned char*)flags.ptr, w_fit, w_reg, v.rbuf(0), v.p[0],
                                               v.rbuf(L & 1), v.Abuf(L & 1), v.p[L & 1], v.delta, aN0, words, (const int*)irregular.ptr, xres.ptr, d, ghost_off, slot0, L, c.stream);
    }
    int resident_status(LaunchCtx& c, int clear, unsigned* pm) override
    {
        const int a = xres.ptr ? thallo_hip_iw_resident_status(xres.ptr, clear, -1, pm, c.stream) : 0;
#ifdef THALLO_RESEARCH
        if (a == 0 && xpst.ptr) return thallo_hip_iw_march_persist_status(xpst.ptr, clear, -1, pm, c.stream);
#endif
        return a;
    }
    void resident_disable() override { resident_ = resident_slab_ = persist_ = false; resident_broken_ = true; }
    bool iter_defers_finish() const override { return true; }
    int pcg_iter_deferred(LaunchCtx& c, SolverVectors& v, int cur, int mode, thallo_sum_t aN, thallo_sum_t aN2, thallo_sum_t aD2, const thallo_prev_t& prev,
                          float* out, double* s12_out) override
    {
        const thallo_sum_t none = { nullptr, 0 };
        thallo_iw_iter_t a = iter_block(v, cur, mode, aN, none, none, aN2, aD2, out, s12_out);
        a.prev = &prev;
        return run_iter(c, a);
    }
    int pcg_iter_finish_from(LaunchCtx& c, const float* part, const double* s12p, int count, thallo_sum_t aN, float* aD_word, float* bN_word) override
    {
        TimedLaunch t(c, "PCGScalars");
        return thallo_hip_iw_pcg_iter_finish(part, s12p, count, aN, aD_word, bN_word, c.stream);
    }
    int pcg_step1_mode(LaunchCtx& c, SolverVectors& v, int cur, int mode, thallo_sum_t aN, thallo_sum_t aD, thallo_sum_t bN,
                       thallo_sum_t aN2, thallo_sum_t aD2, float* out) override
    {
        TimedLaunch t(c, "PCGStep1");
        return thallo_hip_iw_pcg_step1(W, H, row0_, row1_, (const float*)cs.ptr, urshape, (const unsigned char*)flags.ptr, w_fit, w_reg,
                                       v.z, v.p[cur], v.p[cur ^ 1], v.delta, v.Ap, mode, aN, aD, bN, aN2, aD2, (const int*)irregular.ptr, v.r, out, c.stream);
    }
    int pcg_step2(LaunchCtx& c, SolverVectors& v, thallo_sum_t aN, thallo_sum_t aD, float* out) override
    {
        TimedLaunch t(c, "PCGStep2");
        return thallo_hip_iw_pcg_step2(W, H, row0_, row1_, (const unsigned char*)flags.ptr, w_fit, w_reg, v.r, v.Ap, v.pre, v.z, aN, aD, (const int*)irregular.ptr, out, c.stream);
    }
};

struct GraphIncidence {
    int N = 0, E = 0;
    DeviceBuffer out_ptr, out_v1, in_ptr, in_edge, in_src;
    long ell_stride = 0;
// ... 798 lines not shown
```

thallo_amd/csrc/solver.cpp:

```cpp
#include "solver.hpp"
#include <stdlib.h>
#include <cmath>
#include <cstdarg>
#include <cstdio>
#include <cstring>

namespace thallo {

static thread_local char g_err[512] = "";
void set_error(const char* fmt, ...)
{
    va_list ap; va_start(ap, fmt); vsnprintf(g_err, sizeof(g_err), fmt, ap); va_end(ap);
    fprintf(stderr, "[thallo] error: %s\n", g_err);
}
const char* last_error() { return g_err; }

hipEvent_t KernelTimer::get_event()
{
    if (!pool_.empty()) { hipEvent_t e = pool_.back(); pool_.pop_back(); return e; }
    hipEvent_t e = nullptr; HIP_OK(hipEventCreate(&e)); return e;
}
int KernelTimer::begin(const char* name, hipStream_t s)
{
    auto it = index_.find(name);
// ... 139 lines not shown
            for (auto& st : kt->stats) if (st.samples) {
                const double mean = st.total_ms / st.samples;
                const double sd = std::sqrt(std::fabs(st.sq_ms / st.samples - mean * mean));
                printf("| %-20s |   %4ld   | %8.3f  |   %8.4f  |   %8.4f   |\n", st.name.c_str(), st.samples, st.total_ms, mean, sd);
            }
        }
        printf("|--------------------------------------------------------------------------|\n");
    }
}

Plan::Plan(EnergyPlugin* pl, const Thallo_InitializationParameters& ip_, bool lm, unsigned* dims_)
    : plugin(pl), ip(ip_), dims(dims_), lm_(lm)
{
    memset(&summary, 0, sizeof(summary));
    v_.n = plugin->n_unknowns();
    v_.n_alloc = thallo_hip_vector_elems(v_.n);
    float** vecs[] = { &v_.delta, &v_.r, &v_.z, &v_.Ap, &v_.pre, &v_.p[0], &v_.p[1] };
    for (float** vp : vecs)
        if (!(*vp = (float*)device_alloc((size_t)v_.n_alloc * sizeof(float)))) return;
    if (scratch_.alloc(64 * sizeof(float))) return;
    ctx.timer = &ktimer;
    timer_.enabled = ip.timingLevel >= 1;
    if (ip.timingLevel >= 2) ktimer.period = 1;
    if (ip.timingLevel >= 3) ktimer.invasive = true;
    if (ensure_slots(sp.lIterations)) return;
    ok_ = true;
}

Plan::~Plan()
{
    hipDeviceSynchronize();
    if (host_words_) { hipHostFree(host_words_); host_words_ = nullptr; }
    for (hipEvent_t e : aux_events_) hipEventDestroy(e);
    if (aux_) hipStreamDestroy(aux_);
    dist_release();
    if (rccl_) { rccl_comm_destroy(rccl_); rccl_ = nullptr; }
    for (auto b : bufs_) delete b;
    delete plugin;
}

DeviceBuffer* Plan::register_buffer() { bufs_.push_back(new DeviceBuffer()); return bufs_.back(); }
void* Plan::device_alloc(size_t bytes) { DeviceBuffer* b = register_buffer(); return b->alloc(bytes) ? nullptr : b->ptr; }

int Plan::ensure_slots(int L)
{
    const int need = 2 * L + 6;
    if (need <= parts_slots_) return 0;
    hipDeviceSynchronize();
    if (parts_.alloc(((size_t)need * THALLO_HIP_MAX_PARTIALS + (size_t)need + 64) * sizeof(float))) { set_error("out of device memory for %d reduction slots (lIterations too large?)", need); return -1; }
    parts_slots_ = need; nb_.assign(need, 1); fin_.assign(need, 0);
    read_ab_switches();
    return 0;
}

const char* env_switch(const char* name)
{
    static const char* const known[] = {
        "THALLO_RESIDENT",
        "THALLO_MARCH",
        "THALLO_DELTA_PLANES",
        "THALLO_DIST_P2P",
        "THALLO_FRONTEND",
        "THALLO_DENSE_JTJ_MAX",
        "THALLO_ENABLE_DIRECT_SOLVE",
    };
    static const char* const ab[][2] = {
        { "THALLO_ONE_KERNEL", "one_kernel" },
        { "THALLO_FIN_IN_KERNEL", "fin_in_kernel" },
        { "THALLO_LM_FOLD_P", "lm_fold_p" },
        { "THALLO_SFS_FUSED", "sfs_fused" },
        { "THALLO_SFS_MARCH", "sfs_march" },
        { "THALLO_BA_RENUMBER", "ba_renumber" },
        { "THALLO_LM_FOLD_STEP", "lm_fold_step" },
        { "THALLO_IW_RESIDENT_FOLD", "iw_resident_fold" },
        { "THALLO_SFS_RESIDENT_FOLD", "sfs_resident_fold" },
        { "THALLO_SFS_PAIR", "sfs_pair" },
        { "THALLO_FRONTEND_AGGREGATE", "frontend_aggregate" },
        { "THALLO_FRONTEND_COMPUTED", "frontend_computed" },
        { "THALLO_FRONTEND_PRELOAD", "frontend_preload" },
        { "THALLO_INC_LANES", "inc_lanes" },
        { "THALLO_DELTA_FIRST_TOUCH", "delta_first_touch" },
        { "THALLO_SCHUR_S_MAX_MB", "schur_s_max_mb" },
        { "THALLO_SCHUR_DENSE_MAX_MB", "schur_dense_max_mb" },
        { "THALLO_PERSIST", "persist" },
    };
    for (const char* k : known) if (!strcmp(k, name)) return getenv(name);
    for (size_t i = 0; i < sizeof(ab) / sizeof(ab[0]); ++i) {
        if (strcmp(ab[i][0], name)) continue;
        static std::string slot[sizeof(ab) / sizeof(ab[0])];
        const char* e = getenv("THALLO_AB");
        if (!e) return nullptr;
        const size_t kl = strlen(ab[i][1]);
        for (const char* t = e; *t; ) {
            while (*t == ',' || *t == ' ') ++t;
            const char* end = t; while (*end && *end != ',' && *end != ' ') ++end;
            if ((size_t)(end - t) > kl && !strncmp(t, ab[i][1], kl) && t[kl] == '=') { slot[i].assign(t + kl + 1, end); return slot[i].c_str(); }
            t = end;
        }
        return nullptr;
    }
    set_error("internal: unknown environment switch %s", name);
    return nullptr;
}

void Plan::read_ab_switches()
{
    auto off = [](const char* name) { const char* e = env_switch(name); return e && e[0] == '0'; };
    one_kernel_    = !off("THALLO_ONE_KERNEL");
    fin_in_kernel_ = !off("THALLO_FIN_IN_KERNEL");
    { const char* e = env_switch("THALLO_FIN_IN_KERNEL"); fin_deferred_ = !(e && e[0]); }
    { const char* e = env_switch("THALLO_DELTA_PLANES"); delta_planes_ = e && e[0] ? atoi(e) : -1; if (delta_planes_ > THALLO_HIP_MAX_UPDATE_TERMS + 1) delta_planes_ = THALLO_HIP_MAX_UPDATE_TERMS + 1;
      if (delta_planes_ < -(THALLO_HIP_MAX_UPDATE_TERMS + 1)) delta_planes_ = -(THALLO_HIP_MAX_UPDATE_TERMS + 1);
      const char* c = e ? strchr(e, ':') : nullptr; aux_async_ = c != nullptr; aux_workgroups_ = c && atoi(c + 1) > 0 ? atoi(c + 1) : 0; }
    batch_delta_   = delta_planes_ != 0;
    lm_fold_p_     = !off("THALLO_LM_FOLD_P");
    lm_fold_step_  = !off("THALLO_LM_FOLD_STEP");
    delta_first_touch_ = !off("THALLO_DELTA_FIRST_TOUCH");
}

void Plan::set_param(const char* name, const void* value)
{
#define SETF(f) if (!strcmp(name, #f)) { sp.f = *(const float*)value; return; }
#define SETI(f) if (!strcmp(name, #f)) { sp.f = *(const int*)value; return; }
    SETF(min_relative_decrease) SETF(min_trust_region_radius) SETF(max_trust_region_radius) SETF(q_tolerance)
    SETF(function_tolerance) SETF(trust_region_radius) SETF(radius_decrease_factor) SETF(min_lm_diagonal)
    SETF(max_lm_diagonal) SETF(max_solver_time_in_seconds)
    SETI(residual_reset_period) SETI(nIter) SETI(nIterations) SETI(lIterations)
#undef SETF
#undef SETI
    if (ip.verbosityLevel > 0) printf("Warning: tried to set nonexistent solver parameter %s\n", name);
}
void Plan::get_param(const char* name, void* value)
{
#define GETF(f) if (!strcmp(name, #f)) { *(float*)value = sp.f; return; }
#define GETI(f) if (!strcmp(name, #f)) { *(int*)value = sp.f; return; }
    GETF(min_relative_decrease) GETF(min_trust_region_radius) GETF(max_trust_region_radius) GETF(q_tolerance)
    GETF(function_tolerance) GETF(trust_region_radius) GETF(radius_decrease_factor) GETF(min_lm_diagonal)
    GETF(max_lm_diagonal) GETF(max_solver_time_in_seconds)
    GETI(residual_reset_period) GETI(nIter) GETI(nIterations) GETI(lIterations)
#undef GETF
#undef GETI
    if (ip.verbosityLevel > 0) printf("Warning: tried to get nonexistent solver parameter %s\n", name);
}

float* Plan::host_words()
{
    if (!host_words_ && hipHostMalloc((void**)&host_words_, 16 * sizeof(float), hipHostMallocDefault) != hipSuccess) { host_words_ = nullptr; (void)hipGetLastError(); }
    return host_words_;
}

float Plan::compute_cost()
{
    if (dist_) return dist_cost();
    const int nb = cost_partials(slot(0));
    if (nb < 0) { set_error("cost kernel launch failed (%d)", nb); return NAN; }
    set_nb(0, nb);
    thallo_hip_finish_sum(sum(0), (float*)scratch_.ptr, ctx.stream);
    float f = 0.0f;
    float* hw = host_words();
    HIP_OK(hipMemcpyAsync(hw ? hw : &f, scratch_.ptr, sizeof(float), hipMemcpyDeviceToHost, ctx.stream));
    HIP_OK(hipStreamSynchronize(ctx.stream));
    if (hw) f = hw[0];
    if (resident_wait_ran_out("the steps since the last cost evaluation are void")) return NAN;
    return f;
}

bool Plan::resident_wait_ran_out(const char* void_what)
{
    if (!resident_used_) return false;
    resident_used_ = false;
    unsigned pm[5] = { 0, 0, 0, 0, 0 };
    if (plugin->resident_status(ctx, 1, pm) == 0) return false;
    plugin->resident_disable();
    set_error("%s: a bounded wait inside the resident PCG kernel ran out (wait kind %u, workgroup %u, wave %u, index %u, tag %u): %s; "
              "the plan runs one launch per PCG iteration from now on (Thallo_ProblemInit and solve again)", plugin->name(), pm[0], pm[1], pm[2], pm[3], pm[4], void_what);
    return true;
}

void Plan::init(void** params)
{
    if (!ok_) return;
    finalized_ = false;
    timer_.cleanup();
    ev_total_ = timer_.start("Total", ctx.stream);
    ready_ = false;
    bool local_ok = true;
    if (plugin->bind(params)) { set_error("%s: parameter binding failed", plugin->name()); local_ok = false; }
    if (local_ok) {
        plugin->unknowns_changed();
        if (plugin->prepare(ctx)) { const std::string why = last_error(); set_error("%s: prepare failed: %s", plugin->name(), why.c_str()); local_ok = false; }
    }
    if (!dist_) { if (!local_ok) return; }
    else {
        dist_->failed = false; dist_->stopped = false;
        const bool need_grid = dist_->form == DistForm::Slab;
        bool all = false;
        if (dist_agree(local_ok && (!need_grid || plugin->slab_grid_ok()), all)) return;
        if (!all) {
            if (local_ok && need_grid && !plugin->slab_grid_ok()) set_error("%s: the row-slab schedule needs UrShape on the unit pixel grid on every rank", plugin->name());
            else if (local_ok) set_error("%s: another rank could not start the solve (its parameters, or UrShape off the unit pixel grid); no rank does", plugin->name());
// ... 8 lines not shown
        if (dist_agree(plugin->resident_slab_ok() && dist_->ghost_off > 0, all)) { ready_ = false; return; }
        dist_->resident_all = all;
        if (dist_agree_defer()) { ready_ = false; return; }
    }
    sp.nIter = 0;
    if (!lm_ && one_kernel_ && plugin->one_kernel_iteration() && !plugin->resident_ok()) { ring_prepare(sp.lIterations); ring_L_ = sp.lIterations; }
    prev_cost_ = compute_cost();
    printf("Initial cost: %g\n", prev_cost_);
}

void Plan::finalize()
{
    prev_cost_ = compute_cost();
    if (ip.verbosityLevel > 0) printf("final cost=%g\n", prev_cost_);
    hipDeviceSynchronize();
    timer_.stop(ev_total_, ctx.stream);
    timer_.evaluate(&summary, ip.verbosityLevel > 0, &ktimer);
    timer_.cleanup();
    finalized_ = true;
}

double Plan::cost()
{
    if (!ok_ || !ready_) return dist_ && dist_->stopped ? (double)NAN : 0.0;
    if (!finalized_) prev_cost_ = compute_cost();
    return (double)prev_cost_;
}

int Plan::step(void** params)
{
    if (!ok_ || !ready_) return 0;
    if (plugin->bind(params)) {
        if (dist_) dist_fail("%s: parameter binding failed", plugin->name());
        else { set_error("%s: parameter binding failed", plugin->name()); return 0; }
    }
    if (!lm_) plugin->unknowns_changed();
    if (sp.nIter >= sp.nIterations) { if (!finalized_) finalize(); return 0; }
    if (sp.lIterations < 0) { set_error("lIterations = %d is negative", sp.lIterations); if (!finalized_) finalize(); return 0; }
    if (ensure_slots(sp.lIterations)) {
        if (dist_) dist_fail("out of device memory for the reduction slots");
        else { if (!finalized_) finalize(); return 0; }
    }
    const int ev_iter = timer_.start("Nonlinear Iteration", ctx.stream);
    bufs_at_step_ = bufs_.size();
    if (dist_ && lm_ && !dist_->runs_lm()) { set_error("distributed: %s runs Gauss-Newton only across ranks", plugin->name()); if (!finalized_) finalize(); return 0; }
    const int rc = lm_ && dist_ && dist_->form == DistForm::Shard ? step_lm_shard(ev_iter) : lm_ ? step_lm(ev_iter) : dist_ ? step_gn_slab(ev_iter) : step_gn(ev_iter);
    if (rc == 1 && sp.max_solver_time_in_seconds > 0.0f && ev_total_ >= 0) {
        hipStream_t s = ctx.stream;
        hipEvent_t q = nullptr; hipEventCreate(&q); hipEventRecord(q, s); hipEventSynchronize(q);
        float ms = 0.0f; hipEventElapsedTime(&ms, timer_.events[ev_total_].start, q); hipEventDestroy(q);
        if (ms / 1000.0f > sp.max_solver_time_in_seconds) { finalize(); return 0; }
    }
    return rc;
}

void Plan::linear_update_tail(int L, bool batched)
{
    const int B = 2;
    hipStream_t s = ctx.stream;
    const auto& imgs = plugin->unknown_images();
    const int jN = B + 2 * (L - 1), jD = jN + 1;
    long off = 0;
    for (size_t k = 0; k < imgs.size(); ++k) {
        TimedLaunch t(ctx, "PCGLinearUpdate");
        const long lo = owned_range(k).lo, len = owned_range(k).len;
        float* X = plugin->unknown_ptr((int)k) + lo;
        const float* dl = v_.delta + off + lo;
        if (L > 1 && batched && ((L - 1) & 1))
            thallo_hip_linear_update2(X, dl, v_.p[cur_ ^ 1] + off + lo, sum(jN - 2), sum(jD - 2), v_.p[cur_] + off + lo, sum(jN), sum(jD), len, s);
        else if (L > 0) thallo_hip_linear_update(X, dl, v_.p[cur_] + off + lo, len, sum(jN), sum(jD), s);
        else            thallo_hip_linear_update(X, dl, nullptr, len, sum(B), sum(B), s);
        off += imgs[k].n_floats;
    }
    plugin->unknowns_written();
}
Plan::Owned Plan::owned_range(size_t u) const
{
    const long n = plugin->unknown_images()[u].n_floats;
    if (!dist_ || dist_->full_vectors()) return { 0, n };
    const long rowlen = n / dist_->Hl;
    return { rowlen * dist_->row0, rowlen * (dist_->row1 - dist_->row0) };
}

bool Plan::gn_begin(int ev_iter, int& ev_lin, bool delta_unset)
{
    hipStream_t s = ctx.stream;
    const int ev_setup = bufs_.size() == bufs_at_step_ ? timer_.start_with(ev_iter, "Nonlinear Setup", s) : timer_.start("Nonlinear Setup", s);
    cur_ = 0;
    SolverVectors v_init = v_;
    if (delta_unset) v_init.delta = nullptr;
    int nb = plugin->pcg_init(ctx, v_init, cur_, slot(2));
    if (nb < 0) { set_error("PCGInit1 launch failed (%d)", nb); return false; }
    if (prior_on() && (nb = prior_init(slot(2))) < 0) { set_error("the prior's launch behind PCGInit1 failed (%d)", nb); return false; }
    const char* what = nullptr;
    if (forms_behind_init() && (nb = forms_setup(gn_shift(), v_.r, slot(2), nb, what)) < 0) { set_error("%s failed (%d)", what, nb); return false; }
    set_nb(2, nb); finish(2);
    ev_lin = timer_.stop_start(ev_setup, "Linear Solve", s);
    return true;
}
int Plan::gn_finish(int L, int ev_lin)
{
    last_l_iters = L;
    return timer_.stop_start(ev_lin, "Nonlinear Finish", ctx.stream);
}
int Plan::gn_end(int ev_fin, int ev_iter)
{
    sp.nIter++;
    timer_.stop_both(ev_fin, ev_iter, ctx.stream);
    return 1;
}

int Plan::step_gn(int ev_iter)
{
    if (plugin->direct_solve()) {
        hipStream_t s = ctx.stream;
        cur_ = 0;
        const int nb = plugin->pcg_init(ctx, v_, cur_, slot(2));
        if (nb < 0) { set_error("PCGInit1 launch failed (%d)", nb); return 0; }
        set_nb(2, nb);
        const int ev_lin = timer_.start("Linear Solve", s);
        if (plugin->solve_direct(ctx, v_) < 0) { const std::string why = last_error(); set_error("direct solve failed: %s", why.c_str()); return 0; }
        timer_.stop(ev_lin, s);
        last_l_iters = 0;
        linear_update_tail(0, false);
        sp.nIter++;
        timer_.stop(ev_iter, s);
        return 1;
    }
    if (schur_on_ || block_on_) return step_gn_blocks(ev_iter);
    if (one_kernel_ && sp.lIterations >= 1 && plugin->resident_ok() && !held_on() && !robust_on() && !prior_on()) return step_gn_resident(ev_iter);
    if (one_kernel_ && plugin->one_kernel_iteration()) return step_gn_one_kernel(ev_iter);
    if (plugin->apply_returns_sums() && !prior_on()) return step_gn_expanded(ev_iter);
    const int L = sp.lIterations, B = 2;
    int ev_lin, nb;
    if (!gn_begin(ev_iter, ev_lin)) return 0;
    const bool batched = plugin->batches_delta() && batch_delta_;
    for (int k = 0; k < L; ++k) {
        const int jN = B + 2 * k, jD = jN + 1, jB = jN + 2;
        const PrevAlpha a = prev_alpha(k);
        if (batched) nb = plugin->pcg_step1_mode(ctx, v_, cur_, THALLO_IW_STEP1_MODE(k, 1), a.aN, a.aD, sum(jN), a.aN2, a.aD2, slot(jD));
        else         nb = gn_step1(k, a, sum(jN), slot(jD));
        if (nb < 0) { set_error("PCGStep1 launch failed (%d)", nb); return 0; }
        set_nb(jD, nb); finish(jD); cur_ ^= 1;
        nb = plugin->pcg_step2(ctx, v_, sum(jN), sum(jD), slot(jB));
        if (nb < 0) { set_error("PCGStep2 launch failed (%d)", nb); return 0; }
        set_nb(jB, nb); finish(jB);
    }
    const int ev_fin = gn_finish(L, ev_lin);
    linear_update_tail(L, batched);
    return gn_end(ev_fin, ev_iter);
}

void Plan::enable_lm(bool on) { lm_ = on; }
void Plan::unknowns_changed()
{
    if (!ok_ || !ready_) return;
    plugin->unknowns_changed();
    if (lm_ && !finalized_) prev_cost_ = compute_cost();
}

int Plan::ensure_lm_vectors()
{
    if (v_.b) return 0;
    float** vecs[] = { &v_.b, &v_.Adelta, &v_.CtC, &v_.SSq, &v_.prevX, &v_.diag };
    for (float** vp : vecs)
        if (!*vp && !(*vp = (float*)device_alloc((size_t)v_.n_alloc * sizeof(float)))) return -1;
    return 0;
}

Plan::GnSchedule Plan::gn_schedule(int L, int n_ring)
{
    const bool defer = plugin->iter_defers_finish();
    if (n_ring >= 2 && defer && L >= 2 && plugin->persist_ok()) return GnSchedule::Persist;
    return defer ? GnSchedule::Deferred : GnSchedule::FinishInLaunch;
}

int Plan::step_gn_one_kernel(int ev_iter)
{
    if (ensure_iter_buffers()) { set_error("out of device memory for the one-kernel schedule"); return 0; }
    const int L = sp.lIterations;
    const int n_ring = ring_planes(L);
    const GnSchedule sched = gn_schedule(L, n_ring);
    const bool async = n_ring >= 2 && aux_async_ && sched != GnSchedule::Persist && aux_stream();
    const bool delta_unset = delta_first_touch_ && n_ring >= 2 && !async && sched != GnSchedule::Persist && plugin->init_takes_null_delta();
    int ev_lin;
    if (!gn_begin(ev_iter, ev_lin, delta_unset)) return 0;
    GnStep st{ L, n_ring < 2 && batch_delta_ && delta_planes_ != 0 && plugin->batches_delta(), PRing(*this, n_ring, async) };
    st.ring.delta_zero = delta_unset;
    bool done = false;
    switch (sched) {
    case GnSchedule::Persist:        done = gn_loop_persist(st); break;
    case GnSchedule::Deferred:       done = gn_loop_deferred(st, L); break;
    case GnSchedule::FinishInLaunch: done = gn_loop_finish_in_launch(st); break;
    }
    if (!done) return 0;
    const int ev_fin = gn_finish(L, ev_lin);
    if (st.ring.on() && L > 0) {
        if (ring_flush(st.ring, L - 1 - THALLO_HIP_MAX_UPDATE_TERMS) || st.ring.wait_for(L)) { set_error("PCGDeltaUpdate launch failed"); return 0; }
        if (!ring_linear_update(st.ring, L, [](int rc) { return rc >= 0; })) { set_error("PCGLinearUpdate launch failed"); return 0; }
        plugin->unknowns_written();
    } else linear_update_tail(L, st.batched);
    return gn_end(ev_fin, ev_iter);
}

int Plan::gn_launch_mode(GnStep& st, int k)
{
    PRing& R = st.ring;
    if (!R.on()) return THALLO_IW_STEP1_MODE(k, st.batched ? 1 : 0);
    if (ring_flush(R, R.flush_due(k))) { set_error("PCGDeltaUpdate launch failed"); return -1; }
    if (R.wait_to_overwrite(k)) { set_error("PCGDeltaUpdate: stream wait failed"); return -1; }
    return R.launch(k, cur_);
}

bool Plan::gn_loop_deferred(GnStep& st, int k_end)
{
    for (int k = 0; k < k_end; ++k) {
        const int jN = 2 + 2 * k, jD = jN + 1, jB = jN + 2;
        const int mode = gn_launch_mode(st, k);
        if (mode < 0) return false;
        const PrevAlpha a = prev_alpha(k);
        const thallo_prev_t prev = { k ? slot(jD - 2) : nullptr, v_.s12buf((k - 1) & 1), st.nb_prev, k ? scal(jD - 2) : nullptr, k ? scal(jB - 2) : nullptr };
        const int nb = plugin->pcg_iter_deferred(ctx, st.ring.vectors(), cur_, mode, a.aN, a.aN2, a.aD2, prev, slot(jD), v_.s12buf(k & 1));
        if (nb < 0) { set_error("PCGIteration launch failed (%d)", nb); return false; }
        if (k) words_done(k - 1);
        set_nb(jD, nb); st.nb_prev = nb; cur_ ^= 1;
        if (k == st.L - 1 && !gn_finish_last(st, k, nb)) return false;
    }
    return true;
}
bool Plan::gn_finish_last(GnStep& st, int k, int nb)
{
    const int jN = 2 + 2 * k, jD = jN + 1, jB = jN + 2;
    if (plugin->pcg_iter_finish_from(ctx, slot(jD), v_.s12buf(k & 1), nb, sum(jN), scal(jD), scal(jB)) < 0) { set_error("PCGScalars launch failed"); return false; }
    words_done(k);
    return true;
}

bool Plan::gn_loop_persist(GnStep& st)
{
    PRing& R = st.ring;
    const int L = st.L, B = 2, n = R.n;
    if (!gn_loop_deferred(st, 1)) return false;
    for (int k = 1; k < L; ) {
        const int m = L - k < n - 1 ? L - k : n - 1, k1 = k + m;
        if (k1 - 1 >= n && R.flushed < k1 - n) { if (ring_flush(R, k - 2) || R.wait_for(k - 2)) { set_error("PCGDeltaUpdate launch failed"); return false; } }
        const int nb = plugin->pcg_persist(ctx, v_, ring_.data(), n, k, k1, slot(0), parts_slots_, B, st.nb_prev, sum(B + 2 * (k - 1)));
        if (nb < 0) { set_error("PCGLoopPersistent launch failed (%d)", nb); return false; }
        resident_used_ = true;
        for (int i = k; i < k1; ++i) words_done(i - 1);
        set_nb(B + 2 * (k1 - 1) + 1, nb); st.nb_prev = nb;
        if (m & 1) cur_ ^= 1;
        k = k1;
        if (k == L && !gn_finish_last(st, L - 1, nb)) return false;
    }
    return true;
}

bool Plan::gn_loop_finish_in_launch(GnStep& st)
{
    for (int k = 0; k < st.L; ++k) {
        const int jN = 2 + 2 * k, jD = jN + 1, jB = jN + 2;
        const int mode = gn_launch_mode(st, k);
        if (mode < 0) return false;
        const PrevAlpha a = prev_alpha(k);
        const int nb = plugin->pcg_iter(ctx, st.ring.vectors(), cur_, mode, a.aN, a.aD, sum(jN), a.aN2, a.aD2, slot(jD),
                                        fin_in_kernel_ ? scal(jD) : nullptr, fin_in_kernel_ ? scal(jB) : nullptr);
        if (nb < 0) { set_error("PCGIteration launch failed (%d)", nb); return false; }
        set_nb(jD, nb); cur_ ^= 1;
        if (!fin_in_kernel_ && plugin->pcg_iter_finish(ctx, v_, slot(jD), nb, sum(jN), scal(jD), scal(jB)) < 0) { set_error("PCGScalars launch failed"); return false; }
        words_done(k);
    }
    return true;
}

bool Plan::PRing::next_batch(int upto, thallo_update_terms_t& T)
{
    T.count = 0;
    for (; flushed <= upto && T.count < THALLO_HIP_MAX_UPDATE_TERMS; ++flushed) {
        T.p[T.count] = plane(flushed); T.alphaN[T.count] = P.sum(2 + 2 * flushed); T.alphaD[T.count] = P.sum(2 + 2 * flushed + 1); ++T.count;
    }
    return T.count > 0;
}
bool Plan::PRing::events(hipEvent_t& words, hipEvent_t& done)
{
    std::vector<hipEvent_t>& ev = P.aux_events_;
    while (n_ev + 2 > ev.size()) { hipEvent_t e = nullptr; if (hipEventCreateWithFlags(&e, hipEventDisableTiming) != hipSuccess) return false; ev.push_back(e); }
    words = ev[n_ev++]; done = ev[n_ev++];
    return true;
}
int Plan::PRing::wait_for(int term)
{
    for (const Sent& q : sent) {
        if (q.upto < synced) continue;
        if (hipStreamWaitEvent(P.ctx.stream, q.done, 0) != hipSuccess) return -1;
        synced = q.upto + 1;
        if (q.upto >= term) break;
    }
    return 0;
}
int Plan::ring_flush(PRing& R, int upto)
{
    hipStream_t s = ctx.stream;
    thallo_update_terms_t T;
    while (R.next_batch(upto, T)) {
        if (!R.async) {
            TimedLaunch t(ctx, "PCGDeltaUpdate");
            if ((R.delta_zero ? thallo_hip_linear_update_n_from_zero : thallo_hip_linear_update_n)(nullptr, v_.delta, T, v_.n_alloc, 0, s) < 0) return -1;
            R.delta_zero = false;
            R.synced = R.flushed;
            continue;
        }
        hipEvent_t words, done;
        if (!R.events(words, done)) return -1;
        if (hipEventRecord(words, s) != hipSuccess || hipStreamWaitEvent(aux_, words, 0) != hipSuccess) return -1;
        LaunchCtx cx = ctx; cx.stream = aux_;
        {   TimedLaunch t(cx, "PCGDeltaUpdate");
            if (thallo_hip_linear_update_n(nullptr, v_.delta, T, v_.n_alloc, aux_workgroups_ > 0 ? aux_workgroups_ : thallo_hip_device_cu_count(), aux_) < 0) return -1; }
        if (hipEventRecord(done, aux_) != hipSuccess) return -1;
        R.sent.push_back(PRing::Sent{ R.flushed - 1, done });
    }
    return 0;
}

bool Plan::aux_stream()
{
    if (aux_) return true;
    if (aux_failed_) return false;
    int lo = 0, hi = 0;
    if (hipDeviceGetStreamPriorityRange(&lo, &hi) != hipSuccess) lo = 0;
    if (hipStreamCreateWithPriority(&aux_, hipStreamNonBlocking, lo) != hipSuccess) { aux_ = nullptr; aux_failed_ = true; (void)hipGetLastError(); return false; }
    return true;
}

bool Plan::ring_possible() const
{
    return plugin->takes_any_p_plane() && (!dist_ || dist_->form == DistForm::Slab);
}
int Plan::ring_wanted(int L) const
{
    if (!ring_possible() || delta_planes_ == 0 || delta_planes_ == 1 || L < 3) return 0;
    const int want = delta_planes_ >= 2 ? delta_planes_ : delta_planes_ <= -2 ? -delta_planes_ : THALLO_HIP_MAX_UPDATE_TERMS + 1;
    return want > L ? L : want;
}
void Plan::ring_prepare(int L)
{
    const int want = ring_wanted(L);
    if (!want) return;
    if (ring_.size() < 2) { ring_.clear(); ring_.push_back(v_.p[1]); ring_.push_back(v_.p[0]); }
    if (want <= (int)ring_.size() || want <= ring_tried_) return;
    ring_tried_ = want;
    const size_t bytes = (size_t)v_.n_alloc * sizeof(float);
    while ((int)ring_.size() < want) {
        size_t free_b = 0, total_b = 0;
        if (delta_planes_ == -1 && (hipMemGetInfo(&free_b, &total_b) != hipSuccess || bytes > free_b / 4 / (size_t)(want - (int)ring_.size()) ||
                                  bytes * (ring_.size() - 1) > ((size_t)32 << 30))) break;
        void* ptr = nullptr;
        if (hipMalloc(&ptr, bytes) != hipSuccess) { (void)hipGetLastError(); break; }
        if (hipMemsetAsync(ptr, 0, bytes, ctx.stream) != hipSuccess) { (void)hipGetLastError(); hipFree(ptr); break; }
        DeviceBuffer* b = register_buffer(); b->ptr = ptr; b->bytes = bytes;
        ring_.push_back((float*)ptr);
    }
}
int Plan::ring_planes(int L)
{
    const int want = ring_wanted(L);
    if (!want) return 0;
    if (L != ring_L_) { ring_prepare(L); ring_L_ = L; }
    if (ring_.size() < 2) return 0;
    const int n = (int)ring_.size() < want ? (int)ring_.size() : want;
    return n >= 3 || want == 2 ? n : 0;
}

int Plan::step_gn_resident(int ev_iter)
{
    if (ensure_iter_buffers()) { set_error("out of device memory for the one-kernel schedule"); return 0; }
    const int L = sp.lIterations, B = 2;
    int ev_lin;
    if (!gn_begin(ev_iter, ev_lin)) return 0;
    const int nb = plugin->pcg_resident(ctx, v_, L, sum(B), scal(B + 1));
    if (nb < 0) { set_error("PCGLoopResident launch failed (%d)", nb); return 0; }
    for (int k = 0; k < L; ++k) { set_nb(B + 2 * k + 1, 1); words_done(k); }
    cur_ = L & 1;
    resident_used_ = true;
    const int ev_fin = gn_finish(L, ev_lin);
    if (plugin->resident_updates_unknowns()) plugin->unknowns_written();
    else linear_update_tail(L, false);
    return gn_end(ev_fin, ev_iter);
}

int Plan::step_gn_expanded(int ev_iter)
{
    if (ensure_sums_buffer()) { set_error("out of device memory for the single-reduction schedule"); return 0; }
    const int L = sp.lIterations, B = 2;
    hipStream_t s = ctx.stream;
    int ev_lin, nb;
    if (!gn_begin(ev_iter, ev_lin)) return 0;
    const bool defer = fin_in_kernel_ && fin_deferred_;
    int nb_prev = 0;
    for (int k = 0; k < L; ++k) {
        const int jN = B + 2 * k, jD = jN + 1, jB = jN + 2;
        {
            TimedLaunch t(ctx, "PCGUpdate");
            int rc;
            if (defer && k > 0) rc = thallo_hip_pcg_update_fin(v_.r, v_.Ap, plugin->use_preconditioner() ? v_.pre : nullptr, v_.p[cur_], v_.p[cur_ ^ 1], v_.delta, v_.n, sum(jN - 2),
                                                               slot(jD - 2), v_.s12, nb_prev, scal(jD - 2), scal(jN), s);
            else rc = thallo_hip_pcg_update(v_.r, v_.Ap, plugin->use_preconditioner() ? v_.pre : nullptr, v_.p[cur_], v_.p[cur_ ^ 1], v_.delta, v_.n, k == 0,
                                            prev_alpha(k).aN, prev_alpha(k).aD, sum(jN), s);
            if (rc < 0) { set_error("PCGUpdate launch failed"); return 0; }
        }
        cur_ ^= 1;
        const thallo_fin_t fin = { sum(jN), fin_in_kernel_ && !defer ? v_.fin_tickets : nullptr, scal(jD), scal(jB) };
        nb = plugin->apply_jtj_sums(ctx, v_, v_.p[cur_], v_.Ap, slot(jD), fin);
        if (nb < 0) { set_error("PCGStep1 launch failed (%d)", nb); return 0; }
        set_nb(jD, nb); nb_prev = nb;
        if (!fin_in_kernel_ || (defer && k == L - 1)) {
            TimedLaunch t(ctx, "PCGScalars");
            if (thallo_hip_pcg_scalars_finish(slot(jD), v_.s12, nb, sum(jN), scal(jD), scal(jB), s) < 0) { set_error("PCGScalars launch failed"); return 0; }
        }
        words_done(k);
    }
    const int ev_fin = gn_finish(L, ev_lin);
    linear_update_tail(L, false);
    return gn_end(ev_fin, ev_iter);
}
// ... 422 lines not shown
```

thallo_amd/csrc/solver.hpp:

```cpp
#pragma once
#include "plugin.hpp"
#include "ba_reduced.hpp"
#include "rccl_transport.hpp"
#include "../../include/Thallo.h"

namespace thallo {

#define HIP_OK(call) do { hipError_t e__ = (call); if (e__ != hipSuccess) set_error("%s failed: %s", #call, hipGetErrorString(e__)); } while (0)

struct SolverParameters {
    float min_relative_decrease = 1e-3f;
    float min_trust_region_radius = 1e-32f;
    float max_trust_region_radius = 1e16f;
    float q_tolerance = 0.0001f;
    float function_tolerance = 0.000001f;
    float trust_region_radius = 1e4f;
    float radius_decrease_factor = 2.0f;
    float min_lm_diagonal = 1e-6f;
    float max_lm_diagonal = 1e32f;
    float max_solver_time_in_seconds = 0.0f;
    int residual_reset_period = 10;
    int nIter = 0;
    int nIterations = 10;
    int lIterations = 10;
// ... 71 lines not shown
    } check;
    bool switched_off = false;
    std::string info;
    bool failed = false;
    bool stopped = false;
    int inject = 0;
};
struct DistPeerInfo;

class Plan {
public:
    Plan(EnergyPlugin* plugin, const Thallo_InitializationParameters& ip, bool lm, unsigned* dims);
    ~Plan();
    bool ok() const { return ok_; }
    bool ready() const { return ok_ && ready_; }

    void init(void** params);
    int  step(void** params);
    double cost();
    void set_param(const char* name, const void* value);
    void get_param(const char* name, void* value);
    int  alpha_beta_trace(float* out_pairs, int cap);
    void unknowns_changed();
    void enable_lm(bool on);
    bool lm() const { return lm_; }
    int  set_preconditioner(int kind);
    int  set_coarse_aggregates(int cameras_per_aggregate, const int* aggregate_of_camera, long n);
    int  coarse_space(long out[4]);
    int  preconditioner_fallbacks();
    const char* schedule_name();
    int  set_linear_solver(int kind);
    int  schur_blocks() const { return schur_assembled() ? (int)reduced()->blocks() : -1; }
    int  schur_held_points();
    int  schur_dense_nonpositive();
    int  set_held_unknowns(int input, const unsigned char* held, long n);
    long held_unknowns() const { return ready_ ? held_count_ : -1; }
    int  set_prior(int input, const float* mean, const float* weight, long n);
    long prior_terms() const { return ready_ ? prior_count_ : -1; }
    int  prior_cost(double* out);
    int  set_robust_loss(int kind, float scale);
    long robust_weights(float* host_out, long n);
    long covariance(void** params, int input, const int* ids, long n, float* host_out, const ThalloX_CovarianceOptions* opt, ThalloX_CovarianceInfo* info);
    int  set_distributed(const ThalloX_Distributed& cfg);
    int  set_ghost_exchange(int n_boundary, const int* boundary_units, int n_ghost, const int* ghost_units, const int* ghost_src_rank, const int* ghost_src_pos);
    int  use_rccl(const unsigned char* id128, int rank, int world);
    const char* distributed_info() const { return dist_ ? dist_->info.c_str() : ""; }
    void rccl_info(int out[3]);
    int  dist_control(int what, int value);
    int  dist_kernel_only(int reps);

    EnergyPlugin* plugin;
    SolverParameters sp;
    Thallo_InitializationParameters ip;
    Thallo_PerformanceSummary summary;
    LaunchCtx ctx;
    KernelTimer ktimer;
    std::vector<float> ab_trace;
    int last_l_iters = 0;
    unsigned* dims;

private:
    bool ok_ = false;
    bool ready_ = false;
    bool lm_ = false;
    bool finalized_ = true;
    float prev_cost_ = 0.0f;
    SolverVectors v_;
    std::vector<DeviceBuffer*> bufs_;
    DeviceBuffer* register_buffer();
    void* device_alloc(size_t bytes);
    DeviceBuffer parts_;
    int parts_slots_ = 0;
    DeviceBuffer scratch_;
    DeviceBuffer trace_;
    std::vector<int> nb_;
    CoarseTimer timer_;
    float* host_words_ = nullptr;
    int ev_total_ = -1;
    size_t bufs_at_step_ = 0;
    int cur_ = 0;

    float* slot(int j) { return (float*)parts_.ptr + (size_t)j * THALLO_HIP_MAX_PARTIALS; }
    std::vector<char> fin_;
    bool fin_in_kernel_ = true, one_kernel_ = true, batch_delta_ = true, lm_fold_p_ = true, lm_fold_step_ = true, delta_first_touch_ = true;
    int delta_planes_ = -1;
    std::vector<float*> ring_;
    bool ring_possible() const;
    int  ring_wanted(int L) const;
    int  ring_planes(int L);
    void ring_prepare(int L);
    int  ring_tried_ = 0, ring_L_ = -1;
    struct PRing {
        Plan& P;
        const int n;
        const bool async;
        bool delta_zero = false;
        int flushed = 0;
        int synced = 0;
        struct Sent { int upto; hipEvent_t done; };
        std::vector<Sent> sent;
        size_t n_ev = 0;
        SolverVectors v;
        PRing(Plan& plan, int planes, bool on_second_stream) : P(plan), n(planes), async(on_second_stream), v(plan.v_) {}
        PRing(const PRing&) = delete;
        ~PRing() { if (!sent.empty()) (void)hipStreamWaitEvent(P.ctx.stream, sent.back().done, 0); }
        bool on() const { return n >= 2; }
        SolverVectors& vectors() { return on() ? v : P.v_; }
        float* plane(int k) const { return k < 0 ? P.v_.p[0] : P.ring_[(size_t)(k % n)]; }
        int  launch(int k, int cur) { v.p[cur] = plane(k - 1); v.p[cur ^ 1] = plane(k); return k == 0 ? 1 : 2; }
        int  flush_due(int k) const { const int chunk = (n - 1) / 2 > 0 ? (n - 1) / 2 : 1; return (async ? k - 1 - flushed >= chunk : (k >= n && flushed < k - n + 1)) ? k - 2 : -1; }
        bool next_batch(int upto, thallo_update_terms_t& T);
        bool events(hipEvent_t& words, hipEvent_t& done);
        int  wait_for(int term);
        int  wait_to_overwrite(int k) { return k >= n && synced < k - n + 1 ? wait_for(k - n) : 0; }
    };
    int  ring_flush(PRing& R, int upto);
    struct Owned { long lo, len; };
    Owned owned_range(size_t u) const;
    template <class Launched> bool ring_linear_update(PRing& R, int L, Launched launched);
    hipStream_t aux_ = nullptr; bool aux_failed_ = false;
    std::vector<hipEvent_t> aux_events_;
    bool aux_async_ = false;
    int aux_workgroups_ = 0;
    bool aux_stream();
    bool fin_deferred_ = true;
    void read_ab_switches();
    float* scal(int j) { return (float*)parts_.ptr + (size_t)parts_slots_ * THALLO_HIP_MAX_PARTIALS + j; }
    thallo_sum_t partial_sum(int j) { thallo_sum_t s; s.partials = slot(j); s.count = nb_[j]; return s; }
    thallo_sum_t sum(int j) { if (fin_[j]) { thallo_sum_t s; s.partials = scal(j); s.count = 1; return s; } return partial_sum(j); }
    void set_nb(int j, int nb) { nb_[j] = nb; fin_[j] = 0; }
    void finish(int j) { if (nb_[j] <= 256) return; thallo_hip_finish_sum(partial_sum(j), scal(j), ctx.stream); fin_[j] = 1; }
    void words_done(int k) { const int jD = 2 + 2 * k + 1, jB = jD + 1; fin_[jD] = 1; set_nb(jB, 1); fin_[jB] = 1; }
    struct PrevAlpha { thallo_sum_t aN, aD, aN2, aD2; };
    PrevAlpha prev_alpha(int k) { const int jN = 2 + 2 * k, jD = jN + 1; return { sum(k ? jN - 2 : jN), sum(k ? jD - 2 : jD), sum(k > 1 ? jN - 4 : jN), sum(k > 1 ? jD - 4 : jD) }; }
    int  ensure_slots(int L);
    int  ensure_iter_buffers();
    int  ensure_sums_buffer();
    int  step_gn_expanded(int ev_iter);
    enum class GnSchedule { Persist, Deferred, FinishInLaunch };
    struct GnStep {
        const int L;
        const bool batched;
        PRing ring;
        int nb_prev = 0;
    };
    int  step_gn_one_kernel(int ev_iter);
    GnSchedule gn_schedule(int L, int n_ring);
    int  gn_launch_mode(GnStep& st, int k);
    bool gn_finish_last(GnStep& st, int k, int nb);
    bool gn_loop_persist(GnStep& st);
    bool gn_loop_deferred(GnStep& st, int k_end);
    bool gn_loop_finish_in_launch(GnStep& st);
    int  step_gn_resident(int ev_iter);
    bool gn_begin(int ev_iter, int& ev_lin, bool delta_unset = false);
    int  gn_finish(int L, int ev_lin);
    int  gn_end(int ev_fin, int ev_iter);
    bool resident_used_ = false;
    bool resident_wait_ran_out(const char* void_what);
    float compute_cost();
    float* host_words();
    int   step_gn(int ev_iter);
    int   forms_prepare();
    bool  refuse_unless_one_gpu_pcg(bool ok, const char* what_needs);
    bool  forms_behind_init() const { return held_on() || schur_on_ || block_on_; }
    int   forms_setup(const float* shift, const float* b, float* rz_out, int nb, const char*& what);
    int   step_gn_blocks(int ev_iter);
    int   read_word(const unsigned* dev);
    std::string schedule_text_;
    std::map<int, std::vector<unsigned char>> held_masks_;
    long held_count_ = -1;
    unsigned char* held_mask_ = nullptr;
    long held_first_ = 0;
    bool  held_on() const { return held_count_ > 0; }
    bool  schur_empty() const { return schur_on_ && held_on() && held_first_ == schur_n_; }
    int   held_prepare();
    int   hold_pcg(float* rz_out);
    struct PriorInput { std::vector<float> mean, weight; };
    std::map<int, PriorInput> prior_inputs_;
    long prior_count_ = -1;
    float *prior_w_ = nullptr, *prior_mu_ = nullptr, *prior_shift_ = nullptr;
    bool  prior_on() const { return prior_count_ > 0; }
    int   prior_prepare();
    const float* gn_shift() const { return prior_on() ? prior_w_ : nullptr; }
    const float* lm_shift() const { return prior_on() ? prior_shift_ : v_.CtC; }
    int   prior_cost_partials(float* out, int onto);
    int   prior_init(float* rz_out);
    int   cost_partials(float* out);
    int   gn_step1(int k, const PrevAlpha& a, thallo_sum_t bN, float* out);
    int   robust_want_ = 0, robust_on_ = 0;
    float robust_want_scale_ = 0.0f, robust_on_scale_ = 0.0f;
    bool  robust_on() const { return ready_ && robust_on_ != 0; }
    bool block_want_ = false, block_on_ = false;
    thallo_block_regions_t block_regions_;
    thallo_block_regions_t precond_regions_;
    float *block_H_ = nullptr, *block_G_ = nullptr;
    unsigned* block_status_ = nullptr;
    int   block_prepare();
    bool coarse_want_ = false;
    int  coarse_k_ = 0;
    std::vector<int> coarse_agg_;
    int   coarse_apply(float* part, int nb, const unsigned* gate);
    bool schur_want_ = false, schur_on_ = false;
    bool schur_explicit_want_ = false;
    bool schur_dense_want_ = false;
    ReducedCameraSystem* reduced() const { return plugin->reduced_system(); }
    bool  schur_assembled() const { return schur_on_ && reduced()->assembled(); }
    bool  schur_dense() const { return schur_on_ && reduced()->dense_n() >= 0; }
    bool  coarse_on() const { return schur_on_ && reduced()->coarse_n() >= 0; }
    bool  schur_dense_step(const float* g);
    void  schur_dense_pivot_error(int index, const char* where);
    long schur_n_ = 0, schur_hp_off_ = 0, schur_pt_off_ = 0;
    float* schur_g_ = nullptr;
    int   schur_prepare();
    enum class LmSchedule { Reference, OneKernel, OneKernelSlab, Resident, Blocks };
    struct GateOff {
        LaunchCtx& c;
        GateOff(LaunchCtx& ctx, const unsigned* gate) : c(ctx) { thallo_hip_lm_set_gate(gate); c.gate = gate; }
        void off() { thallo_hip_lm_set_gate(nullptr); c.gate = nullptr; }
        ~GateOff() { off(); }
    };
    struct LmStep {
        Plan& P;
        hipStream_t s;
        int L, T0, T1, period;
        static constexpr int B = 2, QS = 1;
        bool slab;
        long o, n, oe, ne;
        bool pc, fold_ctc, fold_init;
        float* lmst;
        const unsigned* gate;
        int ev_iter, ev_lin = -1;
        int k_done = 0;
        bool model_cost_done = false;
        bool failed = false;
        bool coll_failed = false;
        LmStep(Plan& plan, int ev_iter);
        bool skip() const { return failed || (slab && P.dist_->failed); }
// ... 112 lines not shown
```

Measured before the change: 18720.

## Trim first-iteration traffic and apply all ring planes in one delta-update pass

The PCG init can now skip writing pre, z and p_prev, and the first march iteration skips loading p_prev and storing Ap when it is not needed, which cuts memory traffic at the head of each nonlinear step. The delta ring is enlarged to up to 128 planes, and a new single kernel folds all stored search directions into the unknowns at the end, replacing repeated flushes of at most 32 terms. The trade-offs are more ring memory and a large kernel-argument table, and the lean path depends on a plugin check that only the image-warping march path currently passes.

New measurement: 19070 (median of 6 runs). 1.02x the previous value.

```diff
diff --git a/include/thallo_hip.h b/include/thallo_hip.h
--- a/include/thallo_hip.h
+++ b/include/thallo_hip.h
@@ -104,6 +104,9 @@
 typedef struct { const float* p[THALLO_HIP_MAX_UPDATE_TERMS]; thallo_sum_t alphaN[THALLO_HIP_MAX_UPDATE_TERMS], alphaD[THALLO_HIP_MAX_UPDATE_TERMS]; int count; } thallo_update_terms_t;
 int thallo_hip_linear_update_n(float* X, float* delta, thallo_update_terms_t terms, long len, int max_workgroups , thallo_stream_t stream);
 int thallo_hip_linear_update_n_from_zero(float* X, float* delta, thallo_update_terms_t terms, long len, int max_workgroups, thallo_stream_t stream);
+#define THALLO_HIP_MAX_STEP_TERMS 128
+typedef struct { const float* p; thallo_sum_t alphaN, alphaD; } thallo_update_term_t;
+int thallo_hip_linear_update_all(float* X, float* delta, const thallo_update_term_t* terms, int count, long len, int max_workgroups, thallo_stream_t stream);
 int thallo_hip_wave64_selftest(unsigned long long* out_ballot, unsigned* out_peers, float* sums4);
 int thallo_hip_finish_sum(thallo_sum_t s, float* out, thallo_stream_t stream);
 int thallo_hip_finish_sum_gated(thallo_sum_t s, float* out, const unsigned* gate, thallo_stream_t stream);
diff --git a/thallo_amd/csrc/energy_image_warping.hip b/thallo_amd/csrc/energy_image_warping.hip
--- a/thallo_amd/csrc/energy_image_warping.hip
+++ b/thallo_amd/csrc/energy_image_warping.hip
@@ -334,7 +334,7 @@
                 ff = mask[pix] == 0.0f ? 1 : 0;
                 if ((gy < g.row0 || gy >= g.row1) && lx >= 1 && lx <= TW) {
                     cs[pix] = make_float2(cc, ss); flags[pix] = ff;
-                    reinterpret_cast<float2*>(p_prev)[pix] = make_float2(0.f, 0.f); p_prev[2 * N + pix] = 0.f;
+                    if (p_prev) { reinterpret_cast<float2*>(p_prev)[pix] = make_float2(0.f, 0.f); p_prev[2 * N + pix] = 0.f; }
                 }
             }
             T.px[idx] = ox; T.py[idx] = oy; T.c[idx] = cc; T.s[idx] = ss; T.ux[idx] = uxx; T.uy[idx] = uyy; T.f[idx] = ff;
@@ -392,10 +392,10 @@
                     reinterpret_cast<float2*>(diag_out)[pix] = make_float2(dgo_raw, dgo_raw); diag_out[2 * N + pix] = dga_raw;
                 }
                 reinterpret_cast<float2*>(r)[pix] = make_float2(rx, ry);  r[2 * N + pix] = ra;
-                reinterpret_cast<float2*>(pre)[pix] = make_float2(mx, my); pre[2 * N + pix] = ma;
+                if (pre) { reinterpret_cast<float2*>(pre)[pix] = make_float2(mx, my); pre[2 * N + pix] = ma; }
                 const float zx = mx * rx, zy = my * ry, zaa = ma * ra;
-                reinterpret_cast<float2*>(z)[pix] = make_float2(zx, zy);  z[2 * N + pix] = zaa;
-                reinterpret_cast<float2*>(p_prev)[pix] = make_float2(0.f, 0.f); p_prev[2 * N + pix] = 0.f;
+                if (z) { reinterpret_cast<float2*>(z)[pix] = make_float2(zx, zy);  z[2 * N + pix] = zaa; }
+                if (p_prev) { reinterpret_cast<float2*>(p_prev)[pix] = make_float2(0.f, 0.f); p_prev[2 * N + pix] = 0.f; }
                 if (delta) { reinterpret_cast<float2*>(delta)[pix] = make_float2(0.f, 0.f);  delta[2 * N + pix] = 0.f; }
                 cs[pix] = make_float2(T.c[i], T.s[i]);
                 flags[pix] = fl;
diff --git a/thallo_amd/csrc/energy_image_warping_march.hip b/thallo_amd/csrc/energy_image_warping_march.hip
--- a/thallo_amd/csrc/energy_image_warping_march.hip
+++ b/thallo_amd/csrc/energy_image_warping_march.hip
@@ -21,7 +21,9 @@
 template <bool FIRST>
 __device__ __forceinline__ void take(Raw<FIRST>& d, const Raw<FIRST>& s)
 {
-    take4(d.ro, s.ro); take2(d.ra, s.ra); take4(d.po, s.po); take2(d.pa, s.pa); take4(d.cs, s.cs); take1(d.f, s.f);
+    take4(d.ro, s.ro); take2(d.ra, s.ra);
+    if (!FIRST) { take4(d.po, s.po); take2(d.pa, s.pa); }
+    take4(d.cs, s.cs); take1(d.f, s.f);
     if (!FIRST) { take4(d.ao, s.ao); take2(d.aa, s.aa); }
 }
 template <int DMODE>
@@ -98,7 +100,7 @@
         const long i2 = (long)tc * W2 + (xc >> 1);
         s.ro = ldf4(ro4 + i2, nt_ra); s.ra = ldf2(ra2 + i2, nt_ra);
         if (!FIRST) { s.ao = ldf4(ao4 + i2, nt_ra); s.aa = ldf2(aa2 + i2, nt_ra); }
-        s.po = ldf4(po4 + i2, nt_pin); s.pa = ldf2(pa2 + i2, nt_pin);
+        if (!FIRST) { s.po = ldf4(po4 + i2, nt_pin); s.pa = ldf2(pa2 + i2, nt_pin); }
         s.cs = ldf4(cs4 + i2, nt_const);
         s.f = nt_const ? __builtin_nontemporal_load(f4 + (i2 >> 1)) : f4[i2 >> 1];
     };
@@ -126,13 +128,14 @@
             rx[1] = __builtin_fmaf(-alpha, s.ao.z, rx[1]); ry[1] = __builtin_fmaf(-alpha, s.ao.w, ry[1]);
             rq[0] = __builtin_fmaf(-alpha, s.aa.x, rq[0]); rq[1] = __builtin_fmaf(-alpha, s.aa.y, rq[1]);
         }
-        const float ppx[2] = { s.po.x, s.po.z }, ppy[2] = { s.po.y, s.po.w }, ppq[2] = { s.pa.x, s.pa.y };
+        const float ppx[2] = { FIRST ? 0.f : s.po.x, FIRST ? 0.f : s.po.z }, ppy[2] = { FIRST ? 0.f : s.po.y, FIRST ? 0.f : s.po.w }, ppq[2] = { FIRST ? 0.f : s.pa.x, FIRST ? 0.f : s.pa.y };
         const unsigned fl = ok ? (s.f >> (((((long)t * W2 + (x0 >> 1)) & 1) != 0) ? 16 : 0)) & 0xffffu : 0u;
         const float2 m0 = lut[fl & 31u], m1 = lut[(fl >> 8) & 31u];
         const float mo[2] = { m0.x, m1.x }, ma[2] = { m0.y, m1.y };
 #pragma unroll
         for (int q = 0; q < 2; ++q) {
-            wn.px[q] = ok ? mo[q] * rx[q] + beta * ppx[q] : 0.f; wn.py[q] = ok ? mo[q] * ry[q] + beta * ppy[q] : 0.f; wn.pa[q] = ok ? ma[q] * rq[q] + beta * ppq[q] : 0.f;
+            if (FIRST) { wn.px[q] = ok ? __builtin_fmaf(mo[q], rx[q], 0.f) : 0.f; wn.py[q] = ok ? __builtin_fmaf(mo[q], ry[q], 0.f) : 0.f; wn.pa[q] = ok ? __builtin_fmaf(ma[q], rq[q], 0.f) : 0.f; }
+            else { wn.px[q] = ok ? mo[q] * rx[q] + beta * ppx[q] : 0.f; wn.py[q] = ok ? mo[q] * ry[q] + beta * ppy[q] : 0.f; wn.pa[q] = ok ? ma[q] * rq[q] + beta * ppq[q] : 0.f; }
             wn.rx[q] = rx[q]; wn.ry[q] = ry[q]; wn.ra[q] = rq[q]; wn.mo[q] = mo[q]; wn.ma[q] = ma[q];
         }
         wn.c[0] = s.cs.x; wn.s[0] = s.cs.y; wn.c[1] = s.cs.z; wn.s[1] = s.cs.w; wn.f = fl;
@@ -166,7 +169,7 @@
             for (int q = 0; q < 2; ++q)
                 iter_sums_pixel(wc.px[q], wc.py[q], wc.pa[q], ax[q], ay[q], av[q], wc.rx[q], wc.ry[q], wc.ra[q], wc.mo[q], wc.ma[q], acc, s0, s1, s2);
             const long i2 = (long)y * W2 + (x0 >> 1);
-            stf4(Ao4 + i2, make_float4(ax[0], ay[0], ax[1], ay[1]), nt_out); stf2(Aa2 + i2, make_float2(av[0], av[1]), nt_out);
+            if (!FIRST || A_out) { stf4(Ao4 + i2, make_float4(ax[0], ay[0], ax[1], ay[1]), nt_out); stf2(Aa2 + i2, make_float2(av[0], av[1]), nt_out); }
             if (DIST) {
 #pragma unroll
                 for (int k = 0; k < 2; ++k) {
@@ -251,7 +254,7 @@
 
 int thallo::launch_march(const thallo_iw_iter_t& a, hipStream_t stream)
 {
-    if ((a.W & 1) || a.W < 2 || !a.Ap_out || (!(a.mode & 1) && !a.Ap_in)) return -(int)hipErrorInvalidValue;
+    if ((a.W & 1) || a.W < 2 || (!a.Ap_out && (!(a.mode & 1) || a.dist)) || (!(a.mode & 1) && !a.Ap_in)) return -(int)hipErrorInvalidValue;
     if (a.dist && a.gs) return -(int)hipErrorNotSupported;
     return !a.dist ? launch_march_as<false>(a, stream) : launch_march_as<true>(a, stream);
 }
diff --git a/thallo_amd/csrc/pcg_kernels.hip b/thallo_amd/csrc/pcg_kernels.hip
--- a/thallo_amd/csrc/pcg_kernels.hip
+++ b/thallo_amd/csrc/pcg_kernels.hip
@@ -515,7 +515,8 @@
 {
     d.x = __builtin_fmaf(a, q.x, d.x); d.y = __builtin_fmaf(a, q.y, d.y); d.z = __builtin_fmaf(a, q.z, d.z); d.w = __builtin_fmaf(a, q.w, d.w);
 }
-__device__ __forceinline__ void apply_terms4(float4& d, int j, long i, const thallo_update_terms_t& T, const float* al)
+template <class Terms>
+__device__ __forceinline__ void apply_terms4(float4& d, int j, long i, const Terms& T, const float* al)
 {
     for (; j + 8 <= T.count; j += 8) {
         float4 q[8];
@@ -578,6 +579,84 @@
         __syncthreads();
         for (long i = i0; i < len; i += stride) {
             if (i != i0) d = ZERO ? 0.0f : delta[i];
+            for (int j = 0; j < T.count; ++j) d = __builtin_fmaf(al[j], T.p[j][i], d);
+            if (X) X[i] = X[i] + d; else delta[i] = d;
+        }
+    }
+}
+
+struct StepTerms {
+    const float* p[THALLO_HIP_MAX_STEP_TERMS]; const float* aN[THALLO_HIP_MAX_STEP_TERMS]; const float* aD[THALLO_HIP_MAX_STEP_TERMS];
+    int cN[THALLO_HIP_MAX_UPDATE_TERMS], cD[THALLO_HIP_MAX_UPDATE_TERMS];
+    int count;
+};
+static_assert(sizeof(StepTerms) + 3 * 8 <= 4096, "the term table has to fit the kernel-argument segment");
+__device__ __forceinline__ void step_alphas(const StepTerms& T, float* __restrict__ al)
+{
+    const int lane = threadIdx.x & (THALLO_WAVE - 1);
+    const int wave = __builtin_amdgcn_readfirstlane((int)(threadIdx.x / THALLO_WAVE));
+    const bool head = lane < T.count && lane < THALLO_HIP_MAX_UPDATE_TERMS;
+    const int jl = head ? lane : 0;
+    const float* pn = T.aN[jl]; const float* pd = T.aD[jl];
+    const int cn = T.cN[jl], cd = T.cD[jl];
+    const bool list = head && !(cn == 1 && cd == 1);
+    if (wave == 0) {
+        constexpr int ROUNDS = THALLO_HIP_MAX_STEP_TERMS / THALLO_WAVE;
+        float n[ROUNDS], d[ROUNDS];
+#pragma unroll
+        for (int u = 0; u < ROUNDS; ++u) {
+            const int j = lane + u * THALLO_WAVE;
+            const bool word = j < T.count && !(u == 0 && list);
+            n[u] = word ? T.aN[j][0] : 0.0f; d[u] = word ? T.aD[j][0] : 1.0f;
+        }
+#pragma unroll
+        for (int u = 0; u < ROUNDS; ++u) {
+            const int j = lane + u * THALLO_WAVE;
+            if (j < T.count && !(u == 0 && list)) al[j] = safe_div<false>(n[u], d[u]);
+        }
+    }
+    unsigned lists = (unsigned)__ballot(list);
+    lists &= 0x11111111u << wave;
+    while (lists) {
+        const int j = __builtin_ctz(lists);
+        lists &= lists - 1;
+        const float2 s = sum_partials_pair(wave_uniform_ptr(pn, j), __builtin_amdgcn_readlane(cn, j), wave_uniform_ptr(pd, j), __builtin_amdgcn_readlane(cd, j));
+        if (lane == 0) al[j] = safe_div<false>(s.x, s.y);
+    }
+}
+template <bool V4>
+__global__ __launch_bounds__(BLOCK) void k_linear_update_all(float* __restrict__ X, float* __restrict__ delta, StepTerms T, long len)
+{
+    __shared__ float al[THALLO_HIP_MAX_STEP_TERMS];
+    const long i0 = (long)blockIdx.x * BLOCK + threadIdx.x, stride = (long)gridDim.x * BLOCK;
+    if (V4) {
+        const long n4 = len >> 2;
+        const bool have = i0 < n4, eight = T.count >= 8;
+        float4 d = make_float4(0.0f, 0.0f, 0.0f, 0.0f), q[8];
+        if (have && eight) {
+#pragma unroll
+            for (int u = 0; u < 8; ++u) q[u] = ldf4(reinterpret_cast<const float4*>(T.p[u]) + i0, true);
+        }
+        step_alphas(T, al);
+        __syncthreads();
+        if (have) {
+            if (eight) {
+#pragma unroll
+                for (int u = 0; u < 8; ++u) fma4(d, al[u], q[u]);
+            }
+            apply_terms4(d, eight ? 8 : 0, i0, T, al);
+            store_update4(X, delta, i0, d);
+        }
+        for (long i = i0 + stride; i < n4; i += stride) {
+            float4 e = make_float4(0.0f, 0.0f, 0.0f, 0.0f);
+            apply_terms4(e, 0, i, T, al);
+            store_update4(X, delta, i, e);
+        }
+    } else {
+        step_alphas(T, al);
+        __syncthreads();
+        for (long i = i0; i < len; i += stride) {
+            float d = 0.0f;
             for (int j = 0; j < T.count; ++j) d = __builtin_fmaf(al[j], T.p[j][i], d);
             if (X) X[i] = X[i] + d; else delta[i] = d;
         }
@@ -1097,6 +1176,28 @@
     return linear_update_n(true, X, delta, terms, len, max_workgroups, stream);
 }
 
+int thallo_hip_linear_update_all(float* X, float* delta, const thallo_update_term_t* terms, int count, long len, int max_workgroups, thallo_stream_t stream)
+{
+    if ((!X && !delta) || len < 0 || count < 0 || count > THALLO_HIP_MAX_STEP_TERMS || (count > 0 && !terms)) return -(int)hipErrorInvalidValue;
+    bool v4 = !(len & 3) && !((uintptr_t)(X ? X : delta) & 15);
+    StepTerms T = {};
+    T.count = count;
+    for (int j = 0; j < count; ++j) {
+        const thallo_update_term_t& t = terms[j];
+        if (!t.p || !t.alphaN.partials || !t.alphaD.partials || t.alphaN.count < 1 || t.alphaD.count < 1) return -(int)hipErrorInvalidValue;
+        if (j < THALLO_HIP_MAX_UPDATE_TERMS) { T.cN[j] = t.alphaN.count; T.cD[j] = t.alphaD.count; }
+        else if (t.alphaN.count != 1 || t.alphaD.count != 1) return -(int)hipErrorInvalidValue;
+        if ((uintptr_t)t.p & 15) v4 = false;
+        T.p[j] = t.p; T.aN[j] = t.alphaN.partials; T.aD[j] = t.alphaD.partials;
+    }
+    if (len == 0) return 0;
+    int grid = flat_grid(v4 ? len >> 2 : len, 2 * cu_count());
+    if (max_workgroups > 0 && grid > max_workgroups) grid = max_workgroups;
+    hipLaunchKernelGGL(v4 ? k_linear_update_all<true> : k_linear_update_all<false>, dim3(grid), dim3(BLOCK), 0, (hipStream_t)stream, X, delta, T, len);
+    int e = check_launch();
+    return e ? e : grid;
+}
+
 int thallo_hip_finish_sum(thallo_sum_t sum, float* out, thallo_stream_t stream)
 {
     hipLaunchKernelGGL(k_finish_sum, dim3(1), dim3(64), 0, (hipStream_t)stream, sum, out);
diff --git a/thallo_amd/csrc/plugin.hpp b/thallo_amd/csrc/plugin.hpp
--- a/thallo_amd/csrc/plugin.hpp
+++ b/thallo_amd/csrc/plugin.hpp
@@ -111,6 +111,7 @@
                           thallo_sum_t aN_prev, thallo_sum_t aD_prev, thallo_sum_t bN_prev, float* alphaD_out) = 0;
     virtual bool batches_delta() const { return false; }
     virtual bool takes_any_p_plane() const { return false; }
+    virtual bool lean_head_ok() const { return false; }
     virtual bool init_takes_null_delta() const { return false; }
     virtual bool persist_ok() const { return false; }
     virtual int pcg_persist(struct LaunchCtx&, SolverVectors&, float* const* planes, int n_planes, int k0, int k1, float* parts, int slots, int B, int nb_prev, thallo_sum_t alphaN_prev) { return -1; }
diff --git a/thallo_amd/csrc/plugins.cpp b/thallo_amd/csrc/plugins.cpp
--- a/thallo_amd/csrc/plugins.cpp
+++ b/thallo_amd/csrc/plugins.cpp
@@ -292,6 +292,7 @@
     }
     bool batches_delta() const override { return true; }
     bool init_takes_null_delta() const override { return true; }
+    bool lean_head_ok() const override { return march_ && march_rc_ && row0_ == 0 && row1_ == H && !persist_; }
     bool takes_any_p_plane() const override { return march_; }
     bool persist_ok() const override { return persist_; }
 #ifdef THALLO_RESEARCH
diff --git a/thallo_amd/csrc/solver.cpp b/thallo_amd/csrc/solver.cpp
--- a/thallo_amd/csrc/solver.cpp
+++ b/thallo_amd/csrc/solver.cpp
@@ -245,6 +245,7 @@
         { "THALLO_DELTA_FIRST_TOUCH", "delta_first_touch" },
         { "THALLO_SCHUR_S_MAX_MB", "schur_s_max_mb" },
         { "THALLO_SCHUR_DENSE_MAX_MB", "schur_dense_max_mb" },
+        { "THALLO_LEAN_HEAD", "lean_head" },
         { "THALLO_PERSIST", "persist" },
     };
     for (const char* k : known) if (!strcmp(k, name)) return getenv(name);
@@ -272,13 +273,14 @@
     one_kernel_    = !off("THALLO_ONE_KERNEL");
     fin_in_kernel_ = !off("THALLO_FIN_IN_KERNEL");
     { const char* e = env_switch("THALLO_FIN_IN_KERNEL"); fin_deferred_ = !(e && e[0]); }
-    { const char* e = env_switch("THALLO_DELTA_PLANES"); delta_planes_ = e && e[0] ? atoi(e) : -1; if (delta_planes_ > THALLO_HIP_MAX_UPDATE_TERMS + 1) delta_planes_ = THALLO_HIP_MAX_UPDATE_TERMS + 1;
-      if (delta_planes_ < -(THALLO_HIP_MAX_UPDATE_TERMS + 1)) delta_planes_ = -(THALLO_HIP_MAX_UPDATE_TERMS + 1);
+    { const char* e = env_switch("THALLO_DELTA_PLANES"); delta_planes_ = e && e[0] ? atoi(e) : -1; if (delta_planes_ > THALLO_HIP_MAX_STEP_TERMS) delta_planes_ = THALLO_HIP_MAX_STEP_TERMS;
+      if (delta_planes_ < -THALLO_HIP_MAX_STEP_TERMS) delta_planes_ = -THALLO_HIP_MAX_STEP_TERMS;
       const char* c = e ? strchr(e, ':') : nullptr; aux_async_ = c != nullptr; aux_workgroups_ = c && atoi(c + 1) > 0 ? atoi(c + 1) : 0; }
     batch_delta_   = delta_planes_ != 0;
     lm_fold_p_     = !off("THALLO_LM_FOLD_P");
     lm_fold_step_  = !off("THALLO_LM_FOLD_STEP");
     delta_first_touch_ = !off("THALLO_DELTA_FIRST_TOUCH");
+    lean_head_     = !off("THALLO_LEAN_HEAD");
 }
 
 void Plan::set_param(const char* name, const void* value)
@@ -453,13 +455,14 @@
     return { rowlen * dist_->row0, rowlen * (dist_->row1 - dist_->row0) };
 }
 
-bool Plan::gn_begin(int ev_iter, int& ev_lin, bool delta_unset)
+bool Plan::gn_begin(int ev_iter, int& ev_lin, bool delta_unset, bool lean)
 {
     hipStream_t s = ctx.stream;
     const int ev_setup = bufs_.size() == bufs_at_step_ ? timer_.start_with(ev_iter, "Nonlinear Setup", s) : timer_.start("Nonlinear Setup", s);
     cur_ = 0;
     SolverVectors v_init = v_;
     if (delta_unset) v_init.delta = nullptr;
+    if (lean) v_init.pre = v_init.z = v_init.p[cur_] = nullptr;
     int nb = plugin->pcg_init(ctx, v_init, cur_, slot(2));
     if (nb < 0) { set_error("PCGInit1 launch failed (%d)", nb); return false; }
     if (prior_on() && (nb = prior_init(slot(2))) < 0) { set_error("the prior's launch behind PCGInit1 failed (%d)", nb); return false; }
@@ -550,14 +553,17 @@
 {
     if (ensure_iter_buffers()) { set_error("out of device memory for the one-kernel schedule"); return 0; }
     const int L = sp.lIterations;
-    const int n_ring = ring_planes(L);
+    int n_ring = ring_planes(L);
+    if (plugin->persist_ok() && n_ring > THALLO_HIP_MAX_UPDATE_TERMS + 1) n_ring = THALLO_HIP_MAX_UPDATE_TERMS + 1;
     const GnSchedule sched = gn_schedule(L, n_ring);
     const bool async = n_ring >= 2 && aux_async_ && sched != GnSchedule::Persist && aux_stream();
     const bool delta_unset = delta_first_touch_ && n_ring >= 2 && !async && sched != GnSchedule::Persist && plugin->init_takes_null_delta();
+    const bool lean = lean_head_ && L >= 2 && sched != GnSchedule::Persist && plugin->lean_head_ok() && !prior_on() && !forms_behind_init() && !held_on() && !robust_on();
     int ev_lin;
-    if (!gn_begin(ev_iter, ev_lin, delta_unset)) return 0;
+    if (!gn_begin(ev_iter, ev_lin, delta_unset, lean)) return 0;
     GnStep st{ L, n_ring < 2 && batch_delta_ && delta_planes_ != 0 && plugin->batches_delta(), PRing(*this, n_ring, async) };
     st.ring.delta_zero = delta_unset;
+    st.lean = lean;
     bool done = false;
     switch (sched) {
     case GnSchedule::Persist:        done = gn_loop_persist(st); break;
@@ -566,7 +572,10 @@
     }
     if (!done) return 0;
     const int ev_fin = gn_finish(L, ev_lin);
-    if (st.ring.on() && L > 0) {
+    if (st.ring.on() && L > 0 && ring_takes_one_pass(st.ring, L)) {
+        if (!ring_step_update(st.ring, L)) { set_error("PCGDeltaUpdate launch failed"); return 0; }
+        plugin->unknowns_written();
+    } else if (st.ring.on() && L > 0) {
         if (ring_flush(st.ring, L - 1 - THALLO_HIP_MAX_UPDATE_TERMS) || st.ring.wait_for(L)) { set_error("PCGDeltaUpdate launch failed"); return 0; }
         if (!ring_linear_update(st.ring, L, [](int rc) { return rc >= 0; })) { set_error("PCGLinearUpdate launch failed"); return 0; }
         plugin->unknowns_written();
@@ -581,6 +590,15 @@
     if (ring_flush(R, R.flush_due(k))) { set_error("PCGDeltaUpdate launch failed"); return -1; }
     if (R.wait_to_overwrite(k)) { set_error("PCGDeltaUpdate: stream wait failed"); return -1; }
     return R.launch(k, cur_);
+}
+
+SolverVectors& Plan::first_launch_vectors(GnStep& st, int k, SolverVectors& v0)
+{
+    SolverVectors& v = st.ring.vectors();
+    if (k != 0 || !st.lean) return v;
+    v0 = v;
+    (cur_ ? v0.Ap : v0.Ap2) = nullptr;
+    return v0;
 }
 
 bool Plan::gn_loop_deferred(GnStep& st, int k_end)
@@ -591,7 +609,8 @@
         if (mode < 0) return false;
         const PrevAlpha a = prev_alpha(k);
         const thallo_prev_t prev = { k ? slot(jD - 2) : nullptr, v_.s12buf((k - 1) & 1), st.nb_prev, k ? scal(jD - 2) : nullptr, k ? scal(jB - 2) : nullptr };
-        const int nb = plugin->pcg_iter_deferred(ctx, st.ring.vectors(), cur_, mode, a.aN, a.aN2, a.aD2, prev, slot(jD), v_.s12buf(k & 1));
+        SolverVectors v0;
+        const int nb = plugin->pcg_iter_deferred(ctx, first_launch_vectors(st, k, v0), cur_, mode, a.aN, a.aN2, a.aD2, prev, slot(jD), v_.s12buf(k & 1));
         if (nb < 0) { set_error("PCGIteration launch failed (%d)", nb); return false; }
         if (k) words_done(k - 1);
         set_nb(jD, nb); st.nb_prev = nb; cur_ ^= 1;
@@ -634,7 +653,8 @@
         const int mode = gn_launch_mode(st, k);
         if (mode < 0) return false;
         const PrevAlpha a = prev_alpha(k);
-        const int nb = plugin->pcg_iter(ctx, st.ring.vectors(), cur_, mode, a.aN, a.aD, sum(jN), a.aN2, a.aD2, slot(jD),
+        SolverVectors v0;
+        const int nb = plugin->pcg_iter(ctx, first_launch_vectors(st, k, v0), cur_, mode, a.aN, a.aD, sum(jN), a.aN2, a.aD2, slot(jD),
                                         fin_in_kernel_ ? scal(jD) : nullptr, fin_in_kernel_ ? scal(jB) : nullptr);
         if (nb < 0) { set_error("PCGIteration launch failed (%d)", nb); return false; }
         set_nb(jD, nb); cur_ ^= 1;
@@ -693,6 +713,28 @@
     return 0;
 }
 
+bool Plan::ring_takes_one_pass(const PRing& R, int L)
+{
+    if (R.async || R.flushed != 0 || L <= 2 * THALLO_HIP_MAX_UPDATE_TERMS || L > THALLO_HIP_MAX_STEP_TERMS) return false;
+    for (int j = THALLO_HIP_MAX_UPDATE_TERMS; j < L; ++j)
+        if (sum(2 + 2 * j).count != 1 || sum(2 + 2 * j + 1).count != 1) return false;
+    return true;
+}
+bool Plan::ring_step_update(PRing& R, int L)
+{
+    thallo_update_term_t T[THALLO_HIP_MAX_STEP_TERMS];
+    long off = 0;
+    for (size_t u = 0; u < plugin->unknown_images().size(); ++u) {
+        TimedLaunch t(ctx, "PCGDeltaUpdate");
+        const Owned o = owned_range(u);
+        for (int j = 0; j < L; ++j) { T[j].p = R.plane(j) + off + o.lo; T[j].alphaN = sum(2 + 2 * j); T[j].alphaD = sum(2 + 2 * j + 1); }
+        if (thallo_hip_linear_update_all(plugin->unknown_ptr((int)u) + o.lo, nullptr, T, L, o.len, 0, ctx.stream) < 0) return false;
+        off += plugin->unknown_images()[u].n_floats;
+    }
+    R.flushed = L;
+    return true;
+}
+
 bool Plan::aux_stream()
 {
     if (aux_) return true;
@@ -710,7 +752,7 @@
 int Plan::ring_wanted(int L) const
 {
     if (!ring_possible() || delta_planes_ == 0 || delta_planes_ == 1 || L < 3) return 0;
-    const int want = delta_planes_ >= 2 ? delta_planes_ : delta_planes_ <= -2 ? -delta_planes_ : THALLO_HIP_MAX_UPDATE_TERMS + 1;
+    const int want = delta_planes_ >= 2 ? delta_planes_ : delta_planes_ <= -2 ? -delta_planes_ : dist_ ? THALLO_HIP_MAX_UPDATE_TERMS + 1 : THALLO_HIP_MAX_STEP_TERMS;
     return want > L ? L : want;
 }
 void Plan::ring_prepare(int L)
diff --git a/thallo_amd/csrc/solver.hpp b/thallo_amd/csrc/solver.hpp
--- a/thallo_amd/csrc/solver.hpp
+++ b/thallo_amd/csrc/solver.hpp
@@ -177,7 +177,7 @@
 
     float* slot(int j) { return (float*)parts_.ptr + (size_t)j * THALLO_HIP_MAX_PARTIALS; }
     std::vector<char> fin_;
-    bool fin_in_kernel_ = true, one_kernel_ = true, batch_delta_ = true, lm_fold_p_ = true, lm_fold_step_ = true, delta_first_touch_ = true;
+    bool fin_in_kernel_ = true, one_kernel_ = true, batch_delta_ = true, lm_fold_p_ = true, lm_fold_step_ = true, delta_first_touch_ = true, lean_head_ = true;
     int delta_planes_ = -1;
     std::vector<float*> ring_;
     bool ring_possible() const;
@@ -210,6 +210,8 @@
         int  wait_to_overwrite(int k) { return k >= n && synced < k - n + 1 ? wait_for(k - n) : 0; }
     };
     int  ring_flush(PRing& R, int upto);
+    bool ring_takes_one_pass(const PRing& R, int L);
+    bool ring_step_update(PRing& R, int L);
     struct Owned { long lo, len; };
     Owned owned_range(size_t u) const;
     template <class Launched> bool ring_linear_update(PRing& R, int L, Launched launched);
@@ -238,7 +240,9 @@
         const bool batched;
         PRing ring;
         int nb_prev = 0;
+        bool lean = false;
     };
+    SolverVectors& first_launch_vectors(GnStep& st, int k, SolverVectors& v0);
     int  step_gn_one_kernel(int ev_iter);
     GnSchedule gn_schedule(int L, int n_ring);
     int  gn_launch_mode(GnStep& st, int k);
@@ -247,7 +251,7 @@
     bool gn_loop_deferred(GnStep& st, int k_end);
     bool gn_loop_finish_in_launch(GnStep& st);
     int  step_gn_resident(int ev_iter);
-    bool gn_begin(int ev_iter, int& ev_lin, bool delta_unset = false);
+    bool gn_begin(int ev_iter, int& ev_lin, bool delta_unset = false, bool lean = false);
     int  gn_finish(int L, int ev_lin);
     int  gn_end(int ev_fin, int ev_iter);
     bool resident_used_ = false;
```
